# tomneda/DABstar

Hardware: AMD Instinct MI355X
Metric: DAB Mode-I ensembles/s (2.048 MS/s IQ->MSC bytes) per GPU; FIB CRC match % (higher is better)
Workload: dtype f32+i32

## Files before the change

dabstar_amd/csrc/vit_t.hip:

```cpp
#include "pipeline.h"
#include "vit_t_gen.h"
#include <vector>

namespace dabx {

__device__ __forceinline__ int bitrev4(int v) { return ((v & 1) << 3) | ((v & 2) << 1) | ((v & 4) >> 1) | ((v & 8) >> 3); }

constexpr int PJB = 32;
constexpr int PCH = 64;
constexpr int PJS = 16 * PCH + 4;
__device__ __forceinline__ int msc_class_of_group(const MscLaunch &L, int g)
{
  int c = 0;
  while (c + 1 < L.n && g >= L.c[c + 1].g0) c++;
  return c;
}

__device__ __forceinline__ uint32_t prep_ld(const uint32_t *p)
{
#if DABX_PREP_NT & 1
  return __builtin_nontemporal_load(p);
#else
  return *p;
#endif
}
__device__ __forceinline__ void prep_st(uint32_t *p, uint32_t v)
{
#if DABX_PREP_NT & 2
  __builtin_nontemporal_store(v, p);
#else
  *p = v;
#endif
}
constexpr int PREP_STG = PJB * 16 * (PCH / 4) / 256;
__device__ __forceinline__ void prep_item(int it, int cw, bool full, int &d, int &pl, int &job)
{
  int jp;
  if (full) { d = it & (PCH / 4 - 1); jp = it / (PCH / 4); }
  else { d = it % cw; jp = it / cw; }
  pl = jp & 15; job = jp >> 4;
}
__device__ __forceinline__ void prep_request(uint32_t (&stage)[PREP_STG], int tid, int p0, int cw, const uint8_t *const *s_base, const long long *s_r,
                                             const int2 *s_mv )
{
  const bool full = cw == PCH / 4;
  if (full) {
    const int pl = (tid >> 4) & 15, d = tid & 15;
    const int brev = bitrev4(pl);
    const unsigned in_plane = (unsigned)pl * (CIF_BITS / 16) + (unsigned)p0 + 4u * (unsigned)d;
#pragma unroll
    for (int r = 0; r < PREP_STG; r++) {
      const uint8_t *base = s_base[r];
      uint32_t v = 0x7F7F7F7Fu;
      if (base) {
        const unsigned slot = (unsigned)(s_r[r] - 16 + brev) & (TDI_SLOTS - 1);
        const int2 mv = s_mv[r];
        v = prep_ld(reinterpret_cast<const uint32_t *>(base + (brev < mv.x ? mv.y : 0) + (size_t)slot * CIF_BITS + in_plane));
      }
      stage[r] = v;
    }
    return;
  }
#pragma unroll
  for (int r = 0; r < PREP_STG; r++) {
    const int it = tid + 256 * r;
    uint32_t v = 0x7F7F7F7Fu;
    if (it < PJB * 16 * cw) {
      int d, pl, job;
      prep_item(it, cw, full, d, pl, job);
      const uint8_t *base = s_base[job];
      if (base) {
        const long long cif = s_r[job] - 16 + bitrev4(pl);
        const int2 mv = s_mv[job];
        v = prep_ld(reinterpret_cast<const uint32_t *>(base + (bitrev4(pl) < mv.x ? mv.y : 0) + (size_t)(cif & (TDI_SLOTS - 1)) * CIF_BITS + (size_t)pl * (CIF_BITS / 16) + p0 + 4 * d));
      }
    }
    stage[r] = v;
  }
}

__global__ __launch_bounds__(256) void k_msc_prep(EngineDev e, int cifs, MscLaunch L)
{
  __builtin_amdgcn_s_setprio(3);
  __shared__ __attribute__((aligned(16))) uint8_t tile[PJB * PJS];
  __shared__ const uint8_t *s_base[PJB];
  __shared__ long long s_r[PJB];
  __shared__ int2 s_mv[PJB];
  const int ci = msc_class_of_group(L, blockIdx.x / (64 / PJB));
  const MscLaunchCls &cl = L.c[ci];
  const int n_in = cl.n_in;
  uint32_t *inT = cl.inT;
  const int tid = threadIdx.x, job0 = (blockIdx.x - cl.g0 * (64 / PJB)) * PJB;
  if (tid < PJB) {
    const MscJob q = msc_class_job(e, cl, job0 + tid, cifs);
    const SubchDev &sc = e.subch[(size_t)q.s * e.max_subch + q.j];
    s_base[tid] = q.valid ? e.tdi + (size_t)q.s * TDI_SLOTS * CIF_BITS + sc.cu_start * 4 : nullptr;
    s_r[tid] = q.r;
    s_mv[tid] = make_int2(q.valid ? msc_move_thr(sc, q.r) : 0, (sc.prev_cu_start - sc.cu_start) * 4);
  }
  const int rows = n_in / 4 + 1;
  const int jl = tid & (PJB - 1), pg = (tid >> 5) & 3, qd = tid >> 7;
  uint32_t *dst = inT + (size_t)(job0 >> 6) * rows * 64 + (job0 & 63) + jl;
  if (pg == 0 && qd == 0) dst[(size_t)(rows - 1) * 64] = 0x7F7F7F7Fu;
  __syncthreads();
  const int npos = n_in / 16;
  uint32_t stage[PREP_STG];
  auto chunk_dwords = [&](int p0) { return (npos - p0 < PCH ? npos - p0 : PCH) / 4; };
  if (npos > 0) prep_request(stage, tid, 0, chunk_dwords(0), s_base, s_r, s_mv);
  for (int p0 = 0; p0 < npos; p0 += PCH) {
    const int cw = chunk_dwords(p0);
    const bool full = cw == PCH / 4;
    if (full) {
      uint8_t *mine_w = tile + ((tid >> 4) & 15) * PCH + 4 * (tid & 15);
#pragma unroll
      for (int r = 0; r < PREP_STG; r++) *reinterpret_cast<uint32_t *>(mine_w + r * PJS) = stage[r];
    } else {
#pragma unroll
      for (int r = 0; r < PREP_STG; r++) {
        const int it = tid + 256 * r;
        if (it < PJB * 16 * cw) {
          int d, pl, job;
          prep_item(it, cw, full, d, pl, job);
          *reinterpret_cast<uint32_t *>(tile + job * PJS + pl * PCH + 4 * d) = stage[r];
        }
      }
    }
    __syncthreads();
    if (p0 + PCH < npos) prep_request(stage, tid, p0 + PCH, chunk_dwords(p0 + PCH), s_base, s_r, s_mv);
    const uint8_t *mine = tile + jl * PJS + (4 * pg) * PCH;
    for (int d = qd; d < cw; d += 2) {
      const uint32_t m0 = *reinterpret_cast<const uint32_t *>(mine + 0 * PCH + 4 * d), m1 = *reinterpret_cast<const uint32_t *>(mine + 1 * PCH + 4 * d);
      const uint32_t m2 = *reinterpret_cast<const uint32_t *>(mine + 2 * PCH + 4 * d), m3 = *reinterpret_cast<const uint32_t *>(mine + 3 * PCH + 4 * d);
      const uint32_t a = __builtin_amdgcn_perm(m1, m0, 0x05010400u), b = __builtin_amdgcn_perm(m1, m0, 0x07030602u);
      const uint32_t c = __builtin_amdgcn_perm(m3, m2, 0x05010400u), f = __builtin_amdgcn_perm(m3, m2, 0x07030602u);
      const int P = p0 + 4 * d;
      prep_st(&dst[(size_t)(4 * (P + 0) + pg) * 64], __builtin_amdgcn_perm(c, a, 0x05040100u));
      prep_st(&dst[(size_t)(4 * (P + 1) + pg) * 64], __builtin_amdgcn_perm(c, a, 0x07060302u));
      prep_st(&dst[(size_t)(4 * (P + 2) + pg) * 64], __builtin_amdgcn_perm(f, b, 0x05040100u));
      prep_st(&dst[(size_t)(4 * (P + 3) + pg) * 64], __builtin_amdgcn_perm(f, b, 0x07060302u));
    }
    __syncthreads();
  }
}

struct VtCycle { uint32_t w[24]; unsigned long long sh; };

typedef unsigned vt_u2 __attribute__((ext_vector_type(2)));
typedef const __attribute__((address_space(4))) vt_u2 *vt_cmap;

typedef __amdgpu_buffer_rsrc_t vt_rsrc;
__device__ __forceinline__ vt_rsrc vt_make_rsrc(const uint32_t *base, unsigned bytes)
{
  return __builtin_amdgcn_make_buffer_rsrc(const_cast<uint32_t *>(base), 0, (int)bytes, 0x00020000);
}
struct VtDec {
  uint2 *p;
#if DABX_VIT_BUF
  vt_rsrc rs;
  int voff;
#endif
};
__device__ __forceinline__ VtDec vt_make_dec(uint2 *group_base, int nsteps, int lane)
{
  VtDec d;
  d.p = group_base + lane;
#if DABX_VIT_BUF
  d.rs = vt_make_rsrc(reinterpret_cast<const uint32_t *>(group_base), (unsigned)nsteps * 512u);
  d.voff = lane * 8;
#else
  (void)nsteps;
#endif
  return d;
}
#ifndef DABX_VIT_ST_AUX
#define DABX_VIT_ST_AUX 2
#define DABX_VIT_LD_AUX 2
#endif
typedef unsigned vt_u2v __attribute__((ext_vector_type(2)));
__device__ __forceinline__ void vt_dec_store(const VtDec &d, int t, unsigned acc0, unsigned acc1)
{
#if DABX_VIT_BUF
  vt_u2v v; v.x = acc0; v.y = acc1;
  __builtin_amdgcn_raw_buffer_store_b64(v, d.rs, d.voff, t * 512, DABX_VIT_ST_AUX);
#elif DABX_VIT_NT & 1
  vt_u2v v; v.x = acc0; v.y = acc1;
  __builtin_nontemporal_store(v, reinterpret_cast<vt_u2v *>(&d.p[(size_t)t * 64]));
#else
  d.p[(size_t)t * 64] = make_uint2(acc0, acc1);
#endif
}
__device__ __forceinline__ uint2 vt_dec_load(const VtDec &d, int t)
{
#if DABX_VIT_BUF
  const vt_u2v v = __builtin_amdgcn_raw_buffer_load_b64(d.rs, d.voff, t * 512, DABX_VIT_LD_AUX);
  return make_uint2(v.x, v.y);
#elif DABX_VIT_NT & 2
  const vt_u2v v = __builtin_nontemporal_load(reinterpret_cast<const vt_u2v *>(&d.p[(size_t)t * 64]));
  return make_uint2(v.x, v.y);
#else
  return d.p[(size_t)t * 64];
#endif
}
#if DABX_VIT_NT & 4
constexpr int VT_IN_AUX = 2;
#else
constexpr int VT_IN_AUX = 0;
#endif
__device__ __forceinline__ void vt_fetch(VtCycle &c, vt_rsrc in_grp, int lane, vt_cmap map, int t0)
{
  c.sh = 0;
#pragma unroll
  for (int s6 = 0; s6 < 6; s6++) {
    const vt_u2 m = map[t0 + s6];
    const unsigned idx[4] = {m.x & 0xFFFFu, m.x >> 16, m.y & 0xFFFFu, m.y >> 16};
#pragma unroll
    for (int p = 0; p < 4; p++) {
      c.w[4 * s6 + p] = (uint32_t)__builtin_amdgcn_raw_buffer_load_b32(in_grp, lane * 4, (int)((idx[p] >> 2) * 256u), VT_IN_AUX);
      c.sh |= (unsigned long long)(idx[p] & 3) << (2 * (4 * s6 + p));
    }
  }
}

template <int TIE> struct VtTie { static constexpr int LIMTOP = 0, REN2 = 0; };
template <> struct VtTie<1> { static constexpr int LIMTOP = 2 * 65535, REN2 = 2 * 60000; };
template <> struct VtTie<2> { static constexpr int LIMTOP = 2 * 32767, REN2 = 2 * 30000; };

template <int C, int TIE = 0, bool CLAMP = false>
__device__ __forceinline__ void vt_one(vt::s2 (&R)[32], const VtCycle &cy, int t, const VtDec &dec_lane, vt::s2 v2n, int &Coff)
{
  unsigned w[4], b[4];
#pragma unroll
  for (int p = 0; p < 4; p++) {
    w[p] = cy.w[4 * C + p];
    b[p] = (unsigned)((cy.sh >> (2 * (4 * C + p))) & 3);
  }
  vt::s2 M[4];
  unsigned acc0, acc1;
  bool pre = false;
  vt::s2 lim = vt::pk(0, 0);
  if constexpr (TIE != 0) {
    if constexpr ((C & 1) != 0) pre = (int)R[0].x + Coff + 1020 * C > VtTie<TIE>::REN2;
    if constexpr (CLAMP) {
      int l = VtTie<TIE>::LIMTOP - Coff - 1020 * (C + 1);
      l = l < 32767 ? l : 32767;
      lim = vt::pk(l, l);
    }
  }
  if constexpr (C == 0) { vt::bm0(w, b, v2n, M); vt::step0<TIE, CLAMP>(R, M, acc0, acc1, lim); }
  else if constexpr (C == 1) { vt::bm1(w, b, v2n, M); vt::step1<TIE, CLAMP>(R, M, acc0, acc1, lim); }
  else if constexpr (C == 2) { vt::bm2(w, b, v2n, M); vt::step2<TIE, CLAMP>(R, M, acc0, acc1, lim); }
  else if constexpr (C == 3) { vt::bm3(w, b, v2n, M); vt::step3<TIE, CLAMP>(R, M, acc0, acc1, lim); }
  else if constexpr (C == 4) { vt::bm4(w, b, v2n, M); vt::step4<TIE, CLAMP>(R, M, acc0, acc1, lim); }
  else { vt::bm5(w, b, v2n, M); vt::step5<TIE, CLAMP>(R, M, acc0, acc1, lim); }
  vt_dec_store(dec_lane, t, acc0, acc1);
  if constexpr (TIE != 0 && (C & 1) != 0) {
    if (__builtin_amdgcn_ballot_w64(pre)) {
      const int mnv = vt::min64(R);
      if (pre) Coff = -mnv - 1020 * (C + 1);
    }
  }
}

template <int TIE, bool CLAMP>
__device__ __forceinline__ void vt_cycle6(vt::s2 (&R)[32], const VtCycle &cy, int t0, const VtDec &dec_lane, vt::s2 v2n, int &Coff)
{
  vt_one<0, TIE, CLAMP>(R, cy, t0 + 0, dec_lane, v2n, Coff);
  vt_one<1, TIE, CLAMP>(R, cy, t0 + 1, dec_lane, v2n, Coff);
  vt_one<2, TIE, CLAMP>(R, cy, t0 + 2, dec_lane, v2n, Coff);
  vt_one<3, TIE, CLAMP>(R, cy, t0 + 3, dec_lane, v2n, Coff);
  vt_one<4, TIE, CLAMP>(R, cy, t0 + 4, dec_lane, v2n, Coff);
  vt_one<5, TIE, CLAMP>(R, cy, t0 + 5, dec_lane, v2n, Coff);
}
template <int TIE, bool ALWAYS_CLAMP>
__device__ __forceinline__ void vt_cycle(vt::s2 (&R)[32], const VtCycle &cy, int t0, const VtDec &dec_lane, vt::s2 v2n, int &Coff)
{
  if constexpr (TIE == 0) vt_cycle6<0, false>(R, cy, t0, dec_lane, v2n, Coff);
  else {
    bool clamp = ALWAYS_CLAMP;
    if constexpr (!ALWAYS_CLAMP) {
      const int room = VtTie<TIE>::LIMTOP - Coff;
      if (__builtin_amdgcn_ballot_w64((int)R[0].x + 14280 + 12240 > room)) {
        const int mxv = vt::max64(R);
        clamp = __builtin_amdgcn_ballot_w64(mxv + 12240 > room) != 0;
      }
    }
    if (clamp) vt_cycle6<TIE, true>(R, cy, t0, dec_lane, v2n, Coff);
    else vt_cycle6<TIE, false>(R, cy, t0, dec_lane, v2n, Coff);
    Coff += 6 * 1020;
  }
}

struct VtDec6 { uint2 w0, w1, w2, w3, w4, w5; };
__device__ __forceinline__ VtDec6 vt_load_dec(const VtDec &dec_lane, int t0)
{
  VtDec6 d;
  d.w0 = vt_dec_load(dec_lane, t0); d.w1 = vt_dec_load(dec_lane, t0 + 1); d.w2 = vt_dec_load(dec_lane, t0 + 2);
  d.w3 = vt_dec_load(dec_lane, t0 + 3); d.w4 = vt_dec_load(dec_lane, t0 + 4); d.w5 = vt_dec_load(dec_lane, t0 + 5);
  return d;
}
template <int C>
__device__ __forceinline__ void vt_back_one(const uint2 w, int t, unsigned &L, unsigned &outw, uint32_t *out, const uint32_t *prbs,
                                            const unsigned char *pos_c)
{
  constexpr unsigned p = 5 - C;
  const unsigned pos = pos_c[L];
  const unsigned long long ww = ((unsigned long long)w.y << 32) | w.x;
  const unsigned bit = (unsigned)(ww >> pos) & 1u;
  const int qb = t - 6;
  outw |= bit << (((qb >> 3) & 3) * 8 + 7 - (qb & 7));
  L = (L & ~(1u << p)) | (bit << p);
  if ((qb & 31) == 0) {
    const unsigned pw = ((const __attribute__((address_space(4))) uint32_t *)(const void *)prbs)[qb >> 5];
    if (out) out[qb >> 5] = outw ^ pw;
    outw = 0;
  }
}

__device__ unsigned long long *g_vt_timeline = nullptr;
__device__ unsigned g_vt_timeline_cap = 0;
__device__ unsigned g_vt_timeline_n = 0;

template <int TIE, bool ALWAYS_CLAMP>
__device__ __forceinline__ void vt_decode(vt_rsrc in_grp, vt_cmap cmap, int nsteps, const VtDec &dec_lane, uint32_t *out, const uint32_t *prbs,
                                          const unsigned char (*pos_tab)[64], int lane, unsigned long long &t_forward_end, bool want_time)
{
  vt::s2 R[32];
#pragma unroll
  for (int r = 0; r < 32; r++) R[r] = vt::pk(2000, 2000);
  R[0] = vt::pk(0, 2000);
  int Coff = 0;
  const int last = nsteps - 6;
  VtCycle ca, cb;
  vt_fetch(ca, in_grp, lane, cmap, 0);
  vt_fetch(cb, in_grp, lane, cmap, 6);
  auto recentre = [&]() {
    const vt::s2 ref = vt::pk(R[0].x, R[0].x);
    if constexpr (TIE != 0) Coff += (int)R[0].x;
#pragma unroll
    for (int r = 0; r < 32; r++) R[r] = R[r] - ref;
  };
  vt::s2 v2n;
  asm volatile("v_mov_b32 %0, %1" : "=v"(v2n) : "s"(0xFFFE0002u));
  int t = 0;
  for (; t + 12 <= nsteps; t += 12) {
    recentre();
    vt_cycle<TIE, ALWAYS_CLAMP>(R, ca, t, dec_lane, v2n, Coff);
    vt_fetch(ca, in_grp, lane, cmap, t + 12 < last ? t + 12 : last);
    vt_cycle<TIE, ALWAYS_CLAMP>(R, cb, t + 6, dec_lane, v2n, Coff);
    vt_fetch(cb, in_grp, lane, cmap, t + 18 < last ? t + 18 : last);
  }
  if (t < nsteps) {
    recentre();
    vt_cycle<TIE, ALWAYS_CLAMP>(R, ca, t, dec_lane, v2n, Coff);
  }
  __builtin_amdgcn_fence(__ATOMIC_RELEASE, "workgroup");
  __builtin_amdgcn_s_waitcnt(0);
  __syncthreads();
  if (want_time) t_forward_end = __builtin_amdgcn_s_memrealtime();

  unsigned L = 0, outw = 0;
  VtDec6 cur = vt_load_dec(dec_lane, nsteps - 6);
  VtDec6 nx1 = vt_load_dec(dec_lane, nsteps - 12);
  for (int tc = nsteps - 6; tc >= 6; tc -= 6) {
    const int tf = tc - 12 > 6 ? tc - 12 : 6;
    const VtDec6 nx2 = vt_load_dec(dec_lane, tf);
    vt_back_one<5>(cur.w5, tc + 5, L, outw, out, prbs, pos_tab[5]);
    vt_back_one<4>(cur.w4, tc + 4, L, outw, out, prbs, pos_tab[4]);
    vt_back_one<3>(cur.w3, tc + 3, L, outw, out, prbs, pos_tab[3]);
    vt_back_one<2>(cur.w2, tc + 2, L, outw, out, prbs, pos_tab[2]);
    vt_back_one<1>(cur.w1, tc + 1, L, outw, out, prbs, pos_tab[1]);
    vt_back_one<0>(cur.w0, tc + 0, L, outw, out, prbs, pos_tab[0]);
    cur = nx1; nx1 = nx2;
  }
}

template <int TIE>
__device__ __forceinline__ void msc_vitT_body(const EngineDev &e, int cifs, const MscLaunch &ML, const uint32_t *prbs)
{
  __shared__ unsigned char pos_tab[6][64];
  const int lane = threadIdx.x;
  unsigned long long *const tl = g_vt_timeline;
  unsigned long long tl0 = 0, tl1 = 0;
  if (tl) tl0 = __builtin_amdgcn_s_memrealtime();
  for (int i = lane; i < 6 * 64; i += 64) pos_tab[i / 64][i % 64] = vt::VT_POS[i / 64][i % 64];
  int gg = blockIdx.x;
  {
    constexpr int ROUND = 1024;
    const int r = gg / ROUND, base = r * ROUND;
    const int len = ML.groups - base < ROUND ? ML.groups - base : ROUND;
    if (r & 1) gg = base + (len - 1 - (gg - base));
  }
  const MscLaunchCls &cl = ML.c[msc_class_of_group(ML, gg)];
  const int g = gg - cl.g0;
  const MscJob q = msc_class_job(e, cl, g * 64 + lane, cifs);
  const int nsteps = cl.nbits + 6, rows = cl.n_in / 4 + 1;
  const vt_rsrc in_grp = vt_make_rsrc(cl.inT + (size_t)g * rows * 64, (unsigned)rows * 256u);
  const VtDec dec_lane = vt_make_dec(cl.decT + (size_t)g * nsteps * 64, nsteps, lane);
  const vt_cmap cmap = (vt_cmap)(const void *)cl.map2;
  uint32_t *out = nullptr;
  if (q.valid)
    out = reinterpret_cast<uint32_t *>(e.msc_out + (((size_t)q.s * e.max_subch + q.j) * MSC_SLOTS + (size_t)(q.out_idx % MSC_SLOTS)) * e.msc_stride);
  vt_decode<TIE, false>(in_grp, cmap, nsteps, dec_lane, out, prbs, pos_tab, lane, tl1, tl != nullptr);
  if (tl && lane == 0) {
    const unsigned slot = atomicAdd(&g_vt_timeline_n, 1u);
    if (slot < g_vt_timeline_cap) {
      unsigned hw, xcc;
      asm volatile("s_getreg_b32 %0, hwreg(HW_REG_HW_ID)" : "=s"(hw));
      asm volatile("s_getreg_b32 %0, hwreg(HW_REG_XCC_ID)" : "=s"(xcc));
      unsigned long long *o = tl + (size_t)slot * 4;
      o[0] = ((unsigned long long)xcc << 32) | hw; o[1] = tl0; o[2] = tl1; o[3] = __builtin_amdgcn_s_memrealtime();
    }
  }
}
#ifdef DABX_VIT_WAVES
#define DABX_VIT_OCC __attribute__((amdgpu_waves_per_eu(DABX_VIT_WAVES, DABX_VIT_WAVES)))
#else
#define DABX_VIT_OCC
#endif
__global__ __launch_bounds__(64) DABX_VIT_OCC void k_msc_vitT(EngineDev e, int cifs, MscLaunch ML, const uint32_t *prbs) { msc_vitT_body<0>(e, cifs, ML, prbs); }
__global__ __launch_bounds__(64) void k_msc_vitT_avx2(EngineDev e, int cifs, MscLaunch ML, const uint32_t *prbs) { msc_vitT_body<1>(e, cifs, ML, prbs); }
__global__ __launch_bounds__(64) void k_msc_vitT_sse2(EngineDev e, int cifs, MscLaunch ML, const uint32_t *prbs) { msc_vitT_body<2>(e, cifs, ML, prbs); }

template <int TIE, bool ALWAYS_CLAMP>
__global__ __launch_bounds__(64) void k_vitT_stage(const uint32_t *symT, const uint16_t *map, int nbits, uint2 *decT, uint32_t *outw, const uint32_t *zeros)
{
  __shared__ unsigned char pos_tab[6][64];
  const int lane = threadIdx.x, g = blockIdx.x;
  for (int i = lane; i < 6 * 64; i += 64) pos_tab[i / 64][i % 64] = vt::VT_POS[i / 64][i % 64];
  const int nsteps = nbits + 6, rows = nsteps + 1;
  const vt_rsrc in_grp = vt_make_rsrc(symT + (size_t)g * rows * 64, (unsigned)rows * 256u);
  unsigned long long unused = 0;
  vt_decode<TIE, ALWAYS_CLAMP>(in_grp, (vt_cmap)(const void *)map, nsteps, vt_make_dec(decT + (size_t)g * nsteps * 64, nsteps, lane),
                               outw + ((size_t)g * 64 + lane) * (nbits / 32), zeros, pos_tab, lane, unused, false);
}

extern "C" int dabx_internal_vitT(const int16_t *soft, int nbits, int batch, int tie_mode, int always_clamp, uint8_t *bits)
{
  if (!soft || !bits || batch <= 0 || nbits < 96 || nbits % 96 != 0 || 4 * (nbits + 6) > 65532 || tie_mode < 0 || tie_mode > 2) {
    set_error("dabx_internal_vitT: bad argument");
    return DABX_E_ARG;
  }
  const int nsteps = nbits + 6, rows = nsteps + 1, groups = (batch + 63) / 64, nw = nbits / 32;
  std::vector<uint32_t> symT((size_t)groups * rows * 64, 0x7F7F7F7Fu);
  for (int b = 0; b < batch; b++)
    for (int r = 0; r < nsteps; r++) {
      uint32_t v = 0;
      for (int k = 0; k < 4; k++) {
        const int16_t sft = soft[(size_t)b * 4 * nsteps + 4 * r + k];
        int sy = tie_mode ? (int)sft + 127 : (int)(int16_t)(sft + 127);
        sy = sy < 0 ? 0 : (sy > 255 ? 255 : sy);
        v |= (uint32_t)sy << (8 * k);
      }
      symT[((size_t)(b / 64) * rows + r) * 64 + (b % 64)] = v;
    }
  std::vector<uint16_t> map((size_t)4 * nsteps + 64);
  for (size_t i = 0; i < map.size(); i++) map[i] = (uint16_t)(i < (size_t)4 * nsteps ? i : 4 * nsteps);
  uint32_t *d_sym = nullptr, *d_out = nullptr, *d_zero = nullptr;
  uint16_t *d_map = nullptr;
  uint2 *d_dec = nullptr;
  int rc = DABX_E_HIP;
  std::vector<uint32_t> outw((size_t)groups * 64 * nw);
  do {
    if (hipMalloc(&d_sym, symT.size() * 4) != hipSuccess || hipMalloc(&d_map, map.size() * 2) != hipSuccess ||
        hipMalloc(&d_dec, (size_t)groups * nsteps * 64 * sizeof(uint2)) != hipSuccess || hipMalloc(&d_out, outw.size() * 4) != hipSuccess ||
        hipMalloc(&d_zero, (size_t)(nw + 1) * 4) != hipSuccess) break;
    if (hipMemcpy(d_sym, symT.data(), symT.size() * 4, hipMemcpyHostToDevice) != hipSuccess) break;
    if (hipMemcpy(d_map, map.data(), map.size() * 2, hipMemcpyHostToDevice) != hipSuccess) break;
    if (hipMemset(d_zero, 0, (size_t)(nw + 1) * 4) != hipSuccess || hipMemset(d_out, 0, outw.size() * 4) != hipSuccess) break;
#define VT_STAGE(T, A) hipLaunchKernelGGL((k_vitT_stage<T, A>), dim3(groups), dim3(64), 0, 0, d_sym, d_map, nbits, d_dec, d_out, d_zero)
    if (tie_mode == 0) VT_STAGE(0, false);
    else if (tie_mode == 1) { if (always_clamp) VT_STAGE(1, true); else VT_STAGE(1, false); }
    else { if (always_clamp) VT_STAGE(2, true); else VT_STAGE(2, false); }
#undef VT_STAGE
    if (hipGetLastError() != hipSuccess || hipDeviceSynchronize() != hipSuccess) break;
    if (hipMemcpy(outw.data(), d_out, outw.size() * 4, hipMemcpyDeviceToHost) != hipSuccess) break;
    rc = 0;
  } while (false);
  (void)hipFree(d_sym); (void)hipFree(d_map); (void)hipFree(d_dec); (void)hipFree(d_out); (void)hipFree(d_zero);
  if (rc) { set_error("dabx_internal_vitT: HIP error"); return rc; }
  for (int b = 0; b < batch; b++) {
    const uint8_t *pb = reinterpret_cast<const uint8_t *>(outw.data() + (size_t)b * nw);
    for (int i = 0; i < nbits; i++) bits[(size_t)b * nbits + i] = (uint8_t)((pb[i >> 3] >> (7 - (i & 7))) & 1);
  }
  return 0;
}

extern "C" int dabx_internal_set_vt_timeline(void *buf, unsigned capacity_records)
{
  unsigned long long *p = reinterpret_cast<unsigned long long *>(buf);
  unsigned zero = 0;
  DABX_HIP(hipMemcpyToSymbol(HIP_SYMBOL(g_vt_timeline_cap), &capacity_records, sizeof(unsigned)));
  DABX_HIP(hipMemcpyToSymbol(HIP_SYMBOL(g_vt_timeline_n), &zero, sizeof(unsigned)));
  DABX_HIP(hipMemcpyToSymbol(HIP_SYMBOL(g_vt_timeline), &p, sizeof(p)));
  return 0;
}

int launch_msc_prep(const EngineDev &e, int cifs, const MscLaunch &L, hipStream_t st, Marker &mk)
{
  mk.begin(6, st);
  hipLaunchKernelGGL(k_msc_prep, dim3(L.groups * (64 / PJB)), dim3(256), 0, st, e, cifs, L);
  mk.end(6, st);
  DABX_HIP(hipGetLastError());
  return 0;
}
int launch_msc_vitT(const EngineDev &e, int cifs, const MscLaunch &L, hipStream_t st, Marker &mk)
{
  const DevTables *t;
  int rc = get_tables(&t);
  if (rc) return rc;
  mk.begin(7, st);
  const int grid = L.groups;
  if (e.tie_mode == 1) hipLaunchKernelGGL(k_msc_vitT_avx2, dim3(grid), dim3(64), 0, st, e, cifs, L, t->prbs_words);
  else if (e.tie_mode == 2) hipLaunchKernelGGL(k_msc_vitT_sse2, dim3(grid), dim3(64), 0, st, e, cifs, L, t->prbs_words);
  else hipLaunchKernelGGL(k_msc_vitT, dim3(grid), dim3(64), 0, st, e, cifs, L, t->prbs_words);
  mk.end(7, st);
  DABX_HIP(hipGetLastError());
  return 0;
}

}
```

dabstar_amd/csrc/vit_t_gen.h:

```cpp
#pragma once
#include <hip/hip_runtime.h>
namespace dabx { namespace vt {
typedef short s2 __attribute__((ext_vector_type(2)));
__device__ __forceinline__ unsigned u(s2 v) { return __builtin_bit_cast(unsigned, v); }
__device__ __forceinline__ s2 s(unsigned v) { return __builtin_bit_cast(s2, v); }
__device__ __forceinline__ s2 pk(int lo, int hi) { return s(__builtin_amdgcn_perm((unsigned)hi, (unsigned)lo, 0x05040100u)); }
__device__ __forceinline__ s2 mn(s2 a, s2 b) { return __builtin_elementwise_min(a, b); }
__device__ __forceinline__ s2 mx(s2 a, s2 b) { return __builtin_elementwise_max(a, b); }
__device__ __forceinline__ int min64(const s2 (&R)[32])
{ s2 a[16];
  for (int i = 0; i < 16; i++) a[i] = mn(R[i], R[i + 16]);
  for (int w = 8; w > 0; w >>= 1) for (int i = 0; i < w; i++) a[i] = mn(a[i], a[i + w]);
  return a[0].x < a[0].y ? (int)a[0].x : (int)a[0].y; }
__device__ __forceinline__ int max64(const s2 (&R)[32])
{ s2 a[16];
  for (int i = 0; i < 16; i++) a[i] = mx(R[i], R[i + 16]);
  for (int w = 8; w > 0; w >>= 1) for (int i = 0; i < w; i++) a[i] = mx(a[i], a[i + w]);
  return a[0].x > a[0].y ? (int)a[0].x : (int)a[0].y; }
__device__ __forceinline__ s2 mn_x(s2 a, s2 b)
{ s2 r; asm("v_pk_min_i16 %0, %1, %2 op_sel:[0,1] op_sel_hi:[1,0]" : "=v"(r) : "v"(a), "v"(b)); return r; }
__device__ __forceinline__ s2 sub_hl(s2 a, s2 b)
{ s2 r; asm("v_pk_sub_i16 %0, %1, %2 op_sel:[1,0] op_sel_hi:[0,1]" : "=v"(r) : "v"(a), "v"(b)); return r; }
__device__ __forceinline__ s2 sub_lh(s2 a, s2 b)
{ s2 r; asm("v_pk_sub_i16 %0, %1, %2 op_sel:[0,1] op_sel_hi:[1,0]" : "=v"(r) : "v"(a), "v"(b)); return r; }
__device__ __forceinline__ unsigned sg(s2 s0, s2 s1) { return __builtin_amdgcn_perm(u(s0), u(s1), 0x0B0A0908u); }
__device__ __forceinline__ unsigned sg_even(s2 dd, s2 ee) { return __builtin_amdgcn_perm(u(dd), u(ee), 0x0C0C090Au); }
__device__ __forceinline__ unsigned sg_odd(s2 dd, s2 ee) { return __builtin_amdgcn_perm(u(dd), u(ee), 0x090A0C0Cu); }
template <int K> __device__ __forceinline__ void fold(unsigned &acc, unsigned p)
{ constexpr unsigned M = 0x01010101u << K;
  if (K == 0) acc = p & M;
  else asm("v_and_or_b32 %0, %1, %2, %0" : "+v"(acc) : "v"(p), "s"(M)); }
__device__ __forceinline__ s2 swap_add(s2 a)
{ s2 r; asm("v_pk_add_u16 %0, %1, %1 op_sel:[0,1] op_sel_hi:[1,0]" : "=v"(r) : "v"(a)); return r; }
__device__ __forceinline__ s2 swap_sub(s2 a) { return sub_lh(a, a); }
__device__ __forceinline__ s2 add_lolo(s2 a, s2 b)
{ s2 r; asm("v_pk_add_u16 %0, %1, %2 op_sel:[0,0] op_sel_hi:[1,0]" : "=v"(r) : "v"(a), "v"(b)); return r; }
__device__ __forceinline__ s2 add_hihi(s2 a, s2 b)
{ s2 r; asm("v_pk_add_u16 %0, %1, %2 op_sel:[0,1] op_sel_hi:[1,1]" : "=v"(r) : "v"(a), "v"(b)); return r; }
__device__ __forceinline__ s2 mad2(s2 a, unsigned k)
{ s2 r; asm("v_pk_mad_i16 %0, %1, 2, %2 op_sel_hi:[1,0,1]" : "=v"(r) : "v"(a), "s"(k)); return r; }
__device__ __forceinline__ s2 madv(s2 a, s2 m, unsigned k)
{ s2 r; asm("v_pk_mad_i16 %0, %1, %2, %3" : "=v"(r) : "v"(a), "v"(m), "s"(k)); return r; }
__device__ __forceinline__ s2 pick(unsigned w_lo, unsigned b_lo, unsigned w_hi, unsigned b_hi)
{ return s(__builtin_amdgcn_perm(w_hi, w_lo, 0x0C000C00u | b_lo | ((4u + b_hi) << 16))); }
constexpr unsigned K_M255 = 0xFF01FF01u, K_M255_P255 = 0x00FFFF01u, K_M510 = 0xFE02FE02u, K_M510_P510 = 0x01FEFE02u;

__device__ constexpr unsigned char VT_P[6] = {5, 4, 3, 2, 1, 0};
__device__ constexpr unsigned char VT_POS[6][64] = {
  {0, 16, 1, 17, 2, 18, 3, 19, 4, 20, 5, 21, 6, 22, 7, 23, 32, 48, 33, 49, 34, 50, 35, 51, 36, 52, 37, 53, 38, 54, 39, 55, 8, 24, 9, 25, 10, 26, 11, 27, 12, 28, 13, 29, 14, 30, 15, 31, 40, 56, 41, 57, 42, 58, 43, 59, 44, 60, 45, 61, 46, 62, 47, 63},
  {16, 17, 18, 19, 20, 21, 22, 23, 48, 49, 50, 51, 52, 53, 54, 55, 0, 1, 2, 3, 4, 5, 6, 7, 32, 33, 34, 35, 36, 37, 38, 39, 24, 25, 26, 27, 28, 29, 30, 31, 56, 57, 58, 59, 60, 61, 62, 63, 8, 9, 10, 11, 12, 13, 14, 15, 40, 41, 42, 43, 44, 45, 46, 47},
  {16, 17, 18, 19, 20, 21, 22, 23, 0, 1, 2, 3, 4, 5, 6, 7, 48, 49, 50, 51, 52, 53, 54, 55, 32, 33, 34, 35, 36, 37, 38, 39, 24, 25, 26, 27, 28, 29, 30, 31, 8, 9, 10, 11, 12, 13, 14, 15, 56, 57, 58, 59, 60, 61, 62, 63, 40, 41, 42, 43, 44, 45, 46, 47},
  {16, 17, 18, 19, 0, 1, 2, 3, 20, 21, 22, 23, 4, 5, 6, 7, 48, 49, 50, 51, 32, 33, 34, 35, 52, 53, 54, 55, 36, 37, 38, 39, 24, 25, 26, 27, 8, 9, 10, 11, 28, 29, 30, 31, 12, 13, 14, 15, 56, 57, 58, 59, 40, 41, 42, 43, 60, 61, 62, 63, 44, 45, 46, 47},
  {16, 17, 0, 1, 18, 19, 2, 3, 20, 21, 4, 5, 22, 23, 6, 7, 48, 49, 32, 33, 50, 51, 34, 35, 52, 53, 36, 37, 54, 55, 38, 39, 24, 25, 8, 9, 26, 27, 10, 11, 28, 29, 12, 13, 30, 31, 14, 15, 56, 57, 40, 41, 58, 59, 42, 43, 60, 61, 44, 45, 62, 63, 46, 47},
  {16, 0, 17, 1, 18, 2, 19, 3, 20, 4, 21, 5, 22, 6, 23, 7, 48, 32, 49, 33, 50, 34, 51, 35, 52, 36, 53, 37, 54, 38, 55, 39, 24, 8, 25, 9, 26, 10, 27, 11, 28, 12, 29, 13, 30, 14, 31, 15, 56, 40, 57, 41, 58, 42, 59, 43, 60, 44, 61, 45, 62, 46, 63, 47},
};

__device__ __forceinline__ void bm0(const unsigned (&w)[4], const unsigned (&b)[4], s2 v2n, s2 (&M)[4])
{
  const s2 A = pick(w[0], b[0], w[3], b[3]);
  const s2 B = pick(w[1], b[1], w[2], b[2]);
  const s2 TS = swap_add(A);
  const s2 Y2 = mad2(TS, K_M510);
  const s2 XB = mad2(B, K_M255);
  const s2 S = swap_add(XB);
  const s2 D = swap_sub(XB);
  M[0] = Y2 + S;
  M[1] = add_lolo(Y2, D);
  M[2] = add_hihi(Y2, D);
  M[3] = Y2 - S;
}
template <int TIE = 0, bool CLAMP = false>
__device__ __forceinline__ void step0(s2 (&R)[32], const s2 (&M)[4], unsigned &acc0, unsigned &acc1, s2 lim = s2{0, 0})
{
  const s2 M0 = M[0];
  const s2 M1 = M[1];
  const s2 M2 = M[2];
  const s2 M3 = M[3];
  s2 t1_0 = R[0] + M0, t2_0 = R[0] - M0;
  if constexpr (CLAMP) { t1_0 = mn(t1_0, lim); t2_0 = mn(t2_0, lim); }
  R[0] = mn_x(t1_0, t2_0);
  s2 t1_1 = R[1] + M3, t2_1 = R[1] - M3;
  if constexpr (CLAMP) { t1_1 = mn(t1_1, lim); t2_1 = mn(t2_1, lim); }
  R[1] = mn_x(t1_1, t2_1);
  if constexpr (TIE == 1) fold<0>(acc0, sg_even(sub_lh(t1_0, t2_0), sub_hl(t2_0, t1_0)) | sg_odd(sub_lh(t1_1, t2_1), sub_hl(t2_1, t1_1)));
  else fold<0>(acc0, sg_even(sub_hl(t2_0, t1_0), sub_lh(t1_0, t2_0)) | sg_odd(sub_hl(t2_1, t1_1), sub_lh(t1_1, t2_1)));
  s2 t1_2 = R[2] - M1, t2_2 = R[2] + M1;
  if constexpr (CLAMP) { t1_2 = mn(t1_2, lim); t2_2 = mn(t2_2, lim); }
  R[2] = mn_x(t1_2, t2_2);
  s2 t1_3 = R[3] - M2, t2_3 = R[3] + M2;
  if constexpr (CLAMP) { t1_3 = mn(t1_3, lim); t2_3 = mn(t2_3, lim); }
  R[3] = mn_x(t1_3, t2_3);
  if constexpr (TIE == 1) fold<1>(acc0, sg_even(sub_lh(t1_2, t2_2), sub_hl(t2_2, t1_2)) | sg_odd(sub_lh(t1_3, t2_3), sub_hl(t2_3, t1_3)));
  else fold<1>(acc0, sg_even(sub_hl(t2_2, t1_2), sub_lh(t1_2, t2_2)) | sg_odd(sub_hl(t2_3, t1_3), sub_lh(t1_3, t2_3)));
  s2 t1_4 = R[4] - M1, t2_4 = R[4] + M1;
  if constexpr (CLAMP) { t1_4 = mn(t1_4, lim); t2_4 = mn(t2_4, lim); }
  R[4] = mn_x(t1_4, t2_4);
  s2 t1_5 = R[5] - M2, t2_5 = R[5] + M2;
  if constexpr (CLAMP) { t1_5 = mn(t1_5, lim); t2_5 = mn(t2_5, lim); }
  R[5] = mn_x(t1_5, t2_5);
  if constexpr (TIE == 1) fold<2>(acc0, sg_even(sub_lh(t1_4, t2_4), sub_hl(t2_4, t1_4)) | sg_odd(sub_lh(t1_5, t2_5), sub_hl(t2_5, t1_5)));
  else fold<2>(acc0, sg_even(sub_hl(t2_4, t1_4), sub_lh(t1_4, t2_4)) | sg_odd(sub_hl(t2_5, t1_5), sub_lh(t1_5, t2_5)));
  s2 t1_6 = R[6] + M0, t2_6 = R[6] - M0;
  if constexpr (CLAMP) { t1_6 = mn(t1_6, lim); t2_6 = mn(t2_6, lim); }
  R[6] = mn_x(t1_6, t2_6);
  s2 t1_7 = R[7] + M3, t2_7 = R[7] - M3;
  if constexpr (CLAMP) { t1_7 = mn(t1_7, lim); t2_7 = mn(t2_7, lim); }
  R[7] = mn_x(t1_7, t2_7);
  if constexpr (TIE == 1) fold<3>(acc0, sg_even(sub_lh(t1_6, t2_6), sub_hl(t2_6, t1_6)) | sg_odd(sub_lh(t1_7, t2_7), sub_hl(t2_7, t1_7)));
  else fold<3>(acc0, sg_even(sub_hl(t2_6, t1_6), sub_lh(t1_6, t2_6)) | sg_odd(sub_hl(t2_7, t1_7), sub_lh(t1_7, t2_7)));
  s2 t1_8 = R[8] + M1, t2_8 = R[8] - M1;
  if constexpr (CLAMP) { t1_8 = mn(t1_8, lim); t2_8 = mn(t2_8, lim); }
  R[8] = mn_x(t1_8, t2_8);
  s2 t1_9 = R[9] + M2, t2_9 = R[9] - M2;
  if constexpr (CLAMP) { t1_9 = mn(t1_9, lim); t2_9 = mn(t2_9, lim); }
  R[9] = mn_x(t1_9, t2_9);
  if constexpr (TIE == 1) fold<4>(acc0, sg_even(sub_lh(t1_8, t2_8), sub_hl(t2_8, t1_8)) | sg_odd(sub_lh(t1_9, t2_9), sub_hl(t2_9, t1_9)));
  else fold<4>(acc0, sg_even(sub_hl(t2_8, t1_8), sub_lh(t1_8, t2_8)) | sg_odd(sub_hl(t2_9, t1_9), sub_lh(t1_9, t2_9)));
  s2 t1_10 = R[10] - M0, t2_10 = R[10] + M0;
  if constexpr (CLAMP) { t1_10 = mn(t1_10, lim); t2_10 = mn(t2_10, lim); }
  R[10] = mn_x(t1_10, t2_10);
  s2 t1_11 = R[11] - M3, t2_11 = R[11] + M3;
  if constexpr (CLAMP) { t1_11 = mn(t1_11, lim); t2_11 = mn(t2_11, lim); }
  R[11] = mn_x(t1_11, t2_11);
  if constexpr (TIE == 1) fold<5>(acc0, sg_even(sub_lh(t1_10, t2_10), sub_hl(t2_10, t1_10)) | sg_odd(sub_lh(t1_11, t2_11), sub_hl(t2_11, t1_11)));
  else fold<5>(acc0, sg_even(sub_hl(t2_10, t1_10), sub_lh(t1_10, t2_10)) | sg_odd(sub_hl(t2_11, t1_11), sub_lh(t1_11, t2_11)));
  s2 t1_12 = R[12] - M0, t2_12 = R[12] + M0;
  if constexpr (CLAMP) { t1_12 = mn(t1_12, lim); t2_12 = mn(t2_12, lim); }
  R[12] = mn_x(t1_12, t2_12);
  s2 t1_13 = R[13] - M3, t2_13 = R[13] + M3;
  if constexpr (CLAMP) { t1_13 = mn(t1_13, lim); t2_13 = mn(t2_13, lim); }
  R[13] = mn_x(t1_13, t2_13);
  if constexpr (TIE == 1) fold<6>(acc0, sg_even(sub_lh(t1_12, t2_12), sub_hl(t2_12, t1_12)) | sg_odd(sub_lh(t1_13, t2_13), sub_hl(t2_13, t1_13)));
  else fold<6>(acc0, sg_even(sub_hl(t2_12, t1_12), sub_lh(t1_12, t2_12)) | sg_odd(sub_hl(t2_13, t1_13), sub_lh(t1_13, t2_13)));
  s2 t1_14 = R[14] + M1, t2_14 = R[14] - M1;
  if constexpr (CLAMP) { t1_14 = mn(t1_14, lim); t2_14 = mn(t2_14, lim); }
  R[14] = mn_x(t1_14, t2_14);
  s2 t1_15 = R[15] + M2, t2_15 = R[15] - M2;
  if constexpr (CLAMP) { t1_15 = mn(t1_15, lim); t2_15 = mn(t2_15, lim); }
  R[15] = mn_x(t1_15, t2_15);
  if constexpr (TIE == 1) fold<7>(acc0, sg_even(sub_lh(t1_14, t2_14), sub_hl(t2_14, t1_14)) | sg_odd(sub_lh(t1_15, t2_15), sub_hl(t2_15, t1_15)));
  else fold<7>(acc0, sg_even(sub_hl(t2_14, t1_14), sub_lh(t1_14, t2_14)) | sg_odd(sub_hl(t2_15, t1_15), sub_lh(t1_15, t2_15)));
  s2 t1_16 = R[16] - M3, t2_16 = R[16] + M3;
  if constexpr (CLAMP) { t1_16 = mn(t1_16, lim); t2_16 = mn(t2_16, lim); }
  R[16] = mn_x(t1_16, t2_16);
  s2 t1_17 = R[17] - M0, t2_17 = R[17] + M0;
  if constexpr (CLAMP) { t1_17 = mn(t1_17, lim); t2_17 = mn(t2_17, lim); }
  R[17] = mn_x(t1_17, t2_17);
  if constexpr (TIE == 1) fold<0>(acc1, sg_even(sub_lh(t1_16, t2_16), sub_hl(t2_16, t1_16)) | sg_odd(sub_lh(t1_17, t2_17), sub_hl(t2_17, t1_17)));
  else fold<0>(acc1, sg_even(sub_hl(t2_16, t1_16), sub_lh(t1_16, t2_16)) | sg_odd(sub_hl(t2_17, t1_17), sub_lh(t1_17, t2_17)));
  s2 t1_18 = R[18] + M2, t2_18 = R[18] - M2;
  if constexpr (CLAMP) { t1_18 = mn(t1_18, lim); t2_18 = mn(t2_18, lim); }
  R[18] = mn_x(t1_18, t2_18);
  s2 t1_19 = R[19] + M1, t2_19 = R[19] - M1;
  if constexpr (CLAMP) { t1_19 = mn(t1_19, lim); t2_19 = mn(t2_19, lim); }
  R[19] = mn_x(t1_19, t2_19);
  if constexpr (TIE == 1) fold<1>(acc1, sg_even(sub_lh(t1_18, t2_18), sub_hl(t2_18, t1_18)) | sg_odd(sub_lh(t1_19, t2_19), sub_hl(t2_19, t1_19)));
  else fold<1>(acc1, sg_even(sub_hl(t2_18, t1_18), sub_lh(t1_18, t2_18)) | sg_odd(sub_hl(t2_19, t1_19), sub_lh(t1_19, t2_19)));
  s2 t1_20 = R[20] + M2, t2_20 = R[20] - M2;
  if constexpr (CLAMP) { t1_20 = mn(t1_20, lim); t2_20 = mn(t2_20, lim); }
  R[20] = mn_x(t1_20, t2_20);
  s2 t1_21 = R[21] + M1, t2_21 = R[21] - M1;
  if constexpr (CLAMP) { t1_21 = mn(t1_21, lim); t2_21 = mn(t2_21, lim); }
  R[21] = mn_x(t1_21, t2_21);
  if constexpr (TIE == 1) fold<2>(acc1, sg_even(sub_lh(t1_20, t2_20), sub_hl(t2_20, t1_20)) | sg_odd(sub_lh(t1_21, t2_21), sub_hl(t2_21, t1_21)));
  else fold<2>(acc1, sg_even(sub_hl(t2_20, t1_20), sub_lh(t1_20, t2_20)) | sg_odd(sub_hl(t2_21, t1_21), sub_lh(t1_21, t2_21)));
  s2 t1_22 = R[22] - M3, t2_22 = R[22] + M3;
  if constexpr (CLAMP) { t1_22 = mn(t1_22, lim); t2_22 = mn(t2_22, lim); }
  R[22] = mn_x(t1_22, t2_22);
  s2 t1_23 = R[23] - M0, t2_23 = R[23] + M0;
  if constexpr (CLAMP) { t1_23 = mn(t1_23, lim); t2_23 = mn(t2_23, lim); }
  R[23] = mn_x(t1_23, t2_23);
  if constexpr (TIE == 1) fold<3>(acc1, sg_even(sub_lh(t1_22, t2_22), sub_hl(t2_22, t1_22)) | sg_odd(sub_lh(t1_23, t2_23), sub_hl(t2_23, t1_23)));
  else fold<3>(acc1, sg_even(sub_hl(t2_22, t1_22), sub_lh(t1_22, t2_22)) | sg_odd(sub_hl(t2_23, t1_23), sub_lh(t1_23, t2_23)));
  s2 t1_24 = R[24] - M2, t2_24 = R[24] + M2;
  if constexpr (CLAMP) { t1_24 = mn(t1_24, lim); t2_24 = mn(t2_24, lim); }
  R[24] = mn_x(t1_24, t2_24);
  s2 t1_25 = R[25] - M1, t2_25 = R[25] + M1;
  if constexpr (CLAMP) { t1_25 = mn(t1_25, lim); t2_25 = mn(t2_25, lim); }
  R[25] = mn_x(t1_25, t2_25);
  if constexpr (TIE == 1) fold<4>(acc1, sg_even(sub_lh(t1_24, t2_24), sub_hl(t2_24, t1_24)) | sg_odd(sub_lh(t1_25, t2_25), sub_hl(t2_25, t1_25)));
  else fold<4>(acc1, sg_even(sub_hl(t2_24, t1_24), sub_lh(t1_24, t2_24)) | sg_odd(sub_hl(t2_25, t1_25), sub_lh(t1_25, t2_25)));
  s2 t1_26 = R[26] + M3, t2_26 = R[26] - M3;
  if constexpr (CLAMP) { t1_26 = mn(t1_26, lim); t2_26 = mn(t2_26, lim); }
  R[26] = mn_x(t1_26, t2_26);
  s2 t1_27 = R[27] + M0, t2_27 = R[27] - M0;
  if constexpr (CLAMP) { t1_27 = mn(t1_27, lim); t2_27 = mn(t2_27, lim); }
  R[27] = mn_x(t1_27, t2_27);
  if constexpr (TIE == 1) fold<5>(acc1, sg_even(sub_lh(t1_26, t2_26), sub_hl(t2_26, t1_26)) | sg_odd(sub_lh(t1_27, t2_27), sub_hl(t2_27, t1_27)));
  else fold<5>(acc1, sg_even(sub_hl(t2_26, t1_26), sub_lh(t1_26, t2_26)) | sg_odd(sub_hl(t2_27, t1_27), sub_lh(t1_27, t2_27)));
  s2 t1_28 = R[28] + M3, t2_28 = R[28] - M3;
  if constexpr (CLAMP) { t1_28 = mn(t1_28, lim); t2_28 = mn(t2_28, lim); }
  R[28] = mn_x(t1_28, t2_28);
  s2 t1_29 = R[29] + M0, t2_29 = R[29] - M0;
  if constexpr (CLAMP) { t1_29 = mn(t1_29, lim); t2_29 = mn(t2_29, lim); }
  R[29] = mn_x(t1_29, t2_29);
  if constexpr (TIE == 1) fold<6>(acc1, sg_even(sub_lh(t1_28, t2_28), sub_hl(t2_28, t1_28)) | sg_odd(sub_lh(t1_29, t2_29), sub_hl(t2_29, t1_29)));
  else fold<6>(acc1, sg_even(sub_hl(t2_28, t1_28), sub_lh(t1_28, t2_28)) | sg_odd(sub_hl(t2_29, t1_29), sub_lh(t1_29, t2_29)));
  s2 t1_30 = R[30] - M2, t2_30 = R[30] + M2;
  if constexpr (CLAMP) { t1_30 = mn(t1_30, lim); t2_30 = mn(t2_30, lim); }
  R[30] = mn_x(t1_30, t2_30);
  s2 t1_31 = R[31] - M1, t2_31 = R[31] + M1;
  if constexpr (CLAMP) { t1_31 = mn(t1_31, lim); t2_31 = mn(t2_31, lim); }
  R[31] = mn_x(t1_31, t2_31);
  if constexpr (TIE == 1) fold<7>(acc1, sg_even(sub_lh(t1_30, t2_30), sub_hl(t2_30, t1_30)) | sg_odd(sub_lh(t1_31, t2_31), sub_hl(t2_31, t1_31)));
  else fold<7>(acc1, sg_even(sub_hl(t2_30, t1_30), sub_lh(t1_30, t2_30)) | sg_odd(sub_hl(t2_31, t1_31), sub_lh(t1_31, t2_31)));
  if constexpr (TIE == 1) { acc0 = ~acc0; acc1 = ~acc1; }
}

__device__ __forceinline__ void bm1(const unsigned (&w)[4], const unsigned (&b)[4], s2 v2n, s2 (&M)[4])
{
  const s2 A = pick(w[0], b[0], w[3], b[3]);
  const s2 U1 = pick(w[1], b[1], w[1], b[1]);
  const s2 U2 = pick(w[2], b[2], w[2], b[2]);
  const s2 TS = swap_add(A);
  const s2 Y2 = mad2(TS, K_M510);
  const s2 X1N = madv(U1, v2n, K_M255_P255);
  const s2 X2N = madv(U2, v2n, K_M255_P255);
  const s2 SN = X1N + X2N;
  const s2 DN = X1N - X2N;
  M[0] = Y2 + SN;
  M[1] = Y2 + DN;
  M[2] = Y2 - SN;
  M[3] = Y2 - DN;
}
template <int TIE = 0, bool CLAMP = false>
__device__ __forceinline__ void step1(s2 (&R)[32], const s2 (&M)[4], unsigned &acc0, unsigned &acc1, s2 lim = s2{0, 0})
{
  const s2 M0 = M[0];
  const s2 M1 = M[1];
  const s2 M2 = M[2];
  const s2 M3 = M[3];
  { s2 a0 = R[0] + M0, b0 = R[16] - M0, a1 = R[0] - M0, b1 = R[16] + M0;
    if constexpr (CLAMP) { a0 = mn(a0, lim); b0 = mn(b0, lim); a1 = mn(a1, lim); b1 = mn(b1, lim); }
    R[0] = mn(a0, b0); R[16] = mn(a1, b1);
    if constexpr (TIE == 1) fold<0>(acc0, sg(a0 - b0, a1 - b1)); else fold<0>(acc0, sg(b0 - a0, b1 - a1)); }
  { s2 a0 = R[1] - M1, b0 = R[17] + M1, a1 = R[1] + M1, b1 = R[17] - M1;
    if constexpr (CLAMP) { a0 = mn(a0, lim); b0 = mn(b0, lim); a1 = mn(a1, lim); b1 = mn(b1, lim); }
    R[1] = mn(a0, b0); R[17] = mn(a1, b1);
    if constexpr (TIE == 1) fold<1>(acc0, sg(a0 - b0, a1 - b1)); else fold<1>(acc0, sg(b0 - a0, b1 - a1)); }
  { s2 a0 = R[2] - M1, b0 = R[18] + M1, a1 = R[2] + M1, b1 = R[18] - M1;
    if constexpr (CLAMP) { a0 = mn(a0, lim); b0 = mn(b0, lim); a1 = mn(a1, lim); b1 = mn(b1, lim); }
    R[2] = mn(a0, b0); R[18] = mn(a1, b1);
    if constexpr (TIE == 1) fold<2>(acc0, sg(a0 - b0, a1 - b1)); else fold<2>(acc0, sg(b0 - a0, b1 - a1)); }
  { s2 a0 = R[3] + M0, b0 = R[19] - M0, a1 = R[3] - M0, b1 = R[19] + M0;
    if constexpr (CLAMP) { a0 = mn(a0, lim); b0 = mn(b0, lim); a1 = mn(a1, lim); b1 = mn(b1, lim); }
    R[3] = mn(a0, b0); R[19] = mn(a1, b1);
    if constexpr (TIE == 1) fold<3>(acc0, sg(a0 - b0, a1 - b1)); else fold<3>(acc0, sg(b0 - a0, b1 - a1)); }
  { s2 a0 = R[4] + M1, b0 = R[20] - M1, a1 = R[4] - M1, b1 = R[20] + M1;
    if constexpr (CLAMP) { a0 = mn(a0, lim); b0 = mn(b0, lim); a1 = mn(a1, lim); b1 = mn(b1, lim); }
    R[4] = mn(a0, b0); R[20] = mn(a1, b1);
    if constexpr (TIE == 1) fold<4>(acc0, sg(a0 - b0, a1 - b1)); else fold<4>(acc0, sg(b0 - a0, b1 - a1)); }
  { s2 a0 = R[5] - M0, b0 = R[21] + M0, a1 = R[5] + M0, b1 = R[21] - M0;
    if constexpr (CLAMP) { a0 = mn(a0, lim); b0 = mn(b0, lim); a1 = mn(a1, lim); b1 = mn(b1, lim); }
    R[5] = mn(a0, b0); R[21] = mn(a1, b1);
    if constexpr (TIE == 1) fold<5>(acc0, sg(a0 - b0, a1 - b1)); else fold<5>(acc0, sg(b0 - a0, b1 - a1)); }
  { s2 a0 = R[6] - M0, b0 = R[22] + M0, a1 = R[6] + M0, b1 = R[22] - M0;
    if constexpr (CLAMP) { a0 = mn(a0, lim); b0 = mn(b0, lim); a1 = mn(a1, lim); b1 = mn(b1, lim); }
    R[6] = mn(a0, b0); R[22] = mn(a1, b1);
    if constexpr (TIE == 1) fold<6>(acc0, sg(a0 - b0, a1 - b1)); else fold<6>(acc0, sg(b0 - a0, b1 - a1)); }
  { s2 a0 = R[7] + M1, b0 = R[23] - M1, a1 = R[7] - M1, b1 = R[23] + M1;
    if constexpr (CLAMP) { a0 = mn(a0, lim); b0 = mn(b0, lim); a1 = mn(a1, lim); b1 = mn(b1, lim); }
    R[7] = mn(a0, b0); R[23] = mn(a1, b1);
    if constexpr (TIE == 1) fold<7>(acc0, sg(a0 - b0, a1 - b1)); else fold<7>(acc0, sg(b0 - a0, b1 - a1)); }
  { s2 a0 = R[8] - M2, b0 = R[24] + M2, a1 = R[8] + M2, b1 = R[24] - M2;
    if constexpr (CLAMP) { a0 = mn(a0, lim); b0 = mn(b0, lim); a1 = mn(a1, lim); b1 = mn(b1, lim); }
    R[8] = mn(a0, b0); R[24] = mn(a1, b1);
    if constexpr (TIE == 1) fold<0>(acc1, sg(a0 - b0, a1 - b1)); else fold<0>(acc1, sg(b0 - a0, b1 - a1)); }
  { s2 a0 = R[9] + M3, b0 = R[25] - M3, a1 = R[9] - M3, b1 = R[25] + M3;
    if constexpr (CLAMP) { a0 = mn(a0, lim); b0 = mn(b0, lim); a1 = mn(a1, lim); b1 = mn(b1, lim); }
    R[9] = mn(a0, b0); R[25] = mn(a1, b1);
    if constexpr (TIE == 1) fold<1>(acc1, sg(a0 - b0, a1 - b1)); else fold<1>(acc1, sg(b0 - a0, b1 - a1)); }
  { s2 a0 = R[10] + M3, b0 = R[26] - M3, a1 = R[10] - M3, b1 = R[26] + M3;
    if constexpr (CLAMP) { a0 = mn(a0, lim); b0 = mn(b0, lim); a1 = mn(a1, lim); b1 = mn(b1, lim); }
    R[10] = mn(a0, b0); R[26] = mn(a1, b1);
    if constexpr (TIE == 1) fold<2>(acc1, sg(a0 - b0, a1 - b1)); else fold<2>(acc1, sg(b0 - a0, b1 - a1)); }
  { s2 a0 = R[11] - M2, b0 = R[27] + M2, a1 = R[11] + M2, b1 = R[27] - M2;
    if constexpr (CLAMP) { a0 = mn(a0, lim); b0 = mn(b0, lim); a1 = mn(a1, lim); b1 = mn(b1, lim); }
    R[11] = mn(a0, b0); R[27] = mn(a1, b1);
    if constexpr (TIE == 1) fold<3>(acc1, sg(a0 - b0, a1 - b1)); else fold<3>(acc1, sg(b0 - a0, b1 - a1)); }
  { s2 a0 = R[12] - M3, b0 = R[28] + M3, a1 = R[12] + M3, b1 = R[28] - M3;
    if constexpr (CLAMP) { a0 = mn(a0, lim); b0 = mn(b0, lim); a1 = mn(a1, lim); b1 = mn(b1, lim); }
    R[12] = mn(a0, b0); R[28] = mn(a1, b1);
    if constexpr (TIE == 1) fold<4>(acc1, sg(a0 - b0, a1 - b1)); else fold<4>(acc1, sg(b0 - a0, b1 - a1)); }
  { s2 a0 = R[13] + M2, b0 = R[29] - M2, a1 = R[13] - M2, b1 = R[29] + M2;
    if constexpr (CLAMP) { a0 = mn(a0, lim); b0 = mn(b0, lim); a1 = mn(a1, lim); b1 = mn(b1, lim); }
    R[13] = mn(a0, b0); R[29] = mn(a1, b1);
    if constexpr (TIE == 1) fold<5>(acc1, sg(a0 - b0, a1 - b1)); else fold<5>(acc1, sg(b0 - a0, b1 - a1)); }
  { s2 a0 = R[14] + M2, b0 = R[30] - M2, a1 = R[14] - M2, b1 = R[30] + M2;
    if constexpr (CLAMP) { a0 = mn(a0, lim); b0 = mn(b0, lim); a1 = mn(a1, lim); b1 = mn(b1, lim); }
    R[14] = mn(a0, b0); R[30] = mn(a1, b1);
    if constexpr (TIE == 1) fold<6>(acc1, sg(a0 - b0, a1 - b1)); else fold<6>(acc1, sg(b0 - a0, b1 - a1)); }
  { s2 a0 = R[15] - M3, b0 = R[31] + M3, a1 = R[15] + M3, b1 = R[31] - M3;
    if constexpr (CLAMP) { a0 = mn(a0, lim); b0 = mn(b0, lim); a1 = mn(a1, lim); b1 = mn(b1, lim); }
    R[15] = mn(a0, b0); R[31] = mn(a1, b1);
    if constexpr (TIE == 1) fold<7>(acc1, sg(a0 - b0, a1 - b1)); else fold<7>(acc1, sg(b0 - a0, b1 - a1)); }
  if constexpr (TIE == 1) { acc0 = ~acc0; acc1 = ~acc1; }
}

__device__ __forceinline__ void bm2(const unsigned (&w)[4], const unsigned (&b)[4], s2 v2n, s2 (&M)[4])
{
  const s2 A = pick(w[0], b[0], w[3], b[3]);
  const s2 U1 = pick(w[1], b[1], w[1], b[1]);
  const s2 U2 = pick(w[2], b[2], w[2], b[2]);
  const s2 TS = swap_add(A);
  const s2 YN = madv(TS, v2n, K_M510_P510);
  const s2 X1N = madv(U1, v2n, K_M255_P255);
  const s2 X2 = mad2(U2, K_M255);
  const s2 PN = YN + X1N;
  const s2 QN = YN - X1N;
  M[0] = PN + X2;
  M[1] = PN - X2;
  M[2] = QN - X2;
  M[3] = QN + X2;
}
template <int TIE = 0, bool CLAMP = false>
__device__ __forceinline__ void step2(s2 (&R)[32], const s2 (&M)[4], unsigned &acc0, unsigned &acc1, s2 lim = s2{0, 0})
{
  const s2 M0 = M[0];
  const s2 M1 = M[1];
  const s2 M2 = M[2];
  const s2 M3 = M[3];
  { s2 a0 = R[0] + M0, b0 = R[8] - M0, a1 = R[0] - M0, b1 = R[8] + M0;
    if constexpr (CLAMP) { a0 = mn(a0, lim); b0 = mn(b0, lim); a1 = mn(a1, lim); b1 = mn(b1, lim); }
    R[0] = mn(a0, b0); R[8] = mn(a1, b1);
    if constexpr (TIE == 1) fold<0>(acc0, sg(a0 - b0, a1 - b1)); else fold<0>(acc0, sg(b0 - a0, b1 - a1)); }
  { s2 a0 = R[1] - M1, b0 = R[9] + M1, a1 = R[1] + M1, b1 = R[9] - M1;
    if constexpr (CLAMP) { a0 = mn(a0, lim); b0 = mn(b0, lim); a1 = mn(a1, lim); b1 = mn(b1, lim); }
    R[1] = mn(a0, b0); R[9] = mn(a1, b1);
    if constexpr (TIE == 1) fold<1>(acc0, sg(a0 - b0, a1 - b1)); else fold<1>(acc0, sg(b0 - a0, b1 - a1)); }
  { s2 a0 = R[2] + M1, b0 = R[10] - M1, a1 = R[2] - M1, b1 = R[10] + M1;
    if constexpr (CLAMP) { a0 = mn(a0, lim); b0 = mn(b0, lim); a1 = mn(a1, lim); b1 = mn(b1, lim); }
    R[2] = mn(a0, b0); R[10] = mn(a1, b1);
    if constexpr (TIE == 1) fold<2>(acc0, sg(a0 - b0, a1 - b1)); else fold<2>(acc0, sg(b0 - a0, b1 - a1)); }
  { s2 a0 = R[3] - M0, b0 = R[11] + M0, a1 = R[3] + M0, b1 = R[11] - M0;
    if constexpr (CLAMP) { a0 = mn(a0, lim); b0 = mn(b0, lim); a1 = mn(a1, lim); b1 = mn(b1, lim); }
    R[3] = mn(a0, b0); R[11] = mn(a1, b1);
    if constexpr (TIE == 1) fold<3>(acc0, sg(a0 - b0, a1 - b1)); else fold<3>(acc0, sg(b0 - a0, b1 - a1)); }
  { s2 a0 = R[4] - M2, b0 = R[12] + M2, a1 = R[4] + M2, b1 = R[12] - M2;
    if constexpr (CLAMP) { a0 = mn(a0, lim); b0 = mn(b0, lim); a1 = mn(a1, lim); b1 = mn(b1, lim); }
    R[4] = mn(a0, b0); R[12] = mn(a1, b1);
    if constexpr (TIE == 1) fold<4>(acc0, sg(a0 - b0, a1 - b1)); else fold<4>(acc0, sg(b0 - a0, b1 - a1)); }
  { s2 a0 = R[5] + M3, b0 = R[13] - M3, a1 = R[5] - M3, b1 = R[13] + M3;
    if constexpr (CLAMP) { a0 = mn(a0, lim); b0 = mn(b0, lim); a1 = mn(a1, lim); b1 = mn(b1, lim); }
    R[5] = mn(a0, b0); R[13] = mn(a1, b1);
    if constexpr (TIE == 1) fold<5>(acc0, sg(a0 - b0, a1 - b1)); else fold<5>(acc0, sg(b0 - a0, b1 - a1)); }
  { s2 a0 = R[6] - M3, b0 = R[14] + M3, a1 = R[6] + M3, b1 = R[14] - M3;
    if constexpr (CLAMP) { a0 = mn(a0, lim); b0 = mn(b0, lim); a1 = mn(a1, lim); b1 = mn(b1, lim); }
    R[6] = mn(a0, b0); R[14] = mn(a1, b1);
    if constexpr (TIE == 1) fold<6>(acc0, sg(a0 - b0, a1 - b1)); else fold<6>(acc0, sg(b0 - a0, b1 - a1)); }
  { s2 a0 = R[7] + M2, b0 = R[15] - M2, a1 = R[7] - M2, b1 = R[15] + M2;
    if constexpr (CLAMP) { a0 = mn(a0, lim); b0 = mn(b0, lim); a1 = mn(a1, lim); b1 = mn(b1, lim); }
    R[7] = mn(a0, b0); R[15] = mn(a1, b1);
    if constexpr (TIE == 1) fold<7>(acc0, sg(a0 - b0, a1 - b1)); else fold<7>(acc0, sg(b0 - a0, b1 - a1)); }
  { s2 a0 = R[16] + M2, b0 = R[24] - M2, a1 = R[16] - M2, b1 = R[24] + M2;
    if constexpr (CLAMP) { a0 = mn(a0, lim); b0 = mn(b0, lim); a1 = mn(a1, lim); b1 = mn(b1, lim); }
    R[16] = mn(a0, b0); R[24] = mn(a1, b1);
    if constexpr (TIE == 1) fold<0>(acc1, sg(a0 - b0, a1 - b1)); else fold<0>(acc1, sg(b0 - a0, b1 - a1)); }
  { s2 a0 = R[17] - M3, b0 = R[25] + M3, a1 = R[17] + M3, b1 = R[25] - M3;
    if constexpr (CLAMP) { a0 = mn(a0, lim); b0 = mn(b0, lim); a1 = mn(a1, lim); b1 = mn(b1, lim); }
    R[17] = mn(a0, b0); R[25] = mn(a1, b1);
    if constexpr (TIE == 1) fold<1>(acc1, sg(a0 - b0, a1 - b1)); else fold<1>(acc1, sg(b0 - a0, b1 - a1)); }
  { s2 a0 = R[18] + M3, b0 = R[26] - M3, a1 = R[18] - M3, b1 = R[26] + M3;
    if constexpr (CLAMP) { a0 = mn(a0, lim); b0 = mn(b0, lim); a1 = mn(a1, lim); b1 = mn(b1, lim); }
    R[18] = mn(a0, b0); R[26] = mn(a1, b1);
    if constexpr (TIE == 1) fold<2>(acc1, sg(a0 - b0, a1 - b1)); else fold<2>(acc1, sg(b0 - a0, b1 - a1)); }
  { s2 a0 = R[19] - M2, b0 = R[27] + M2, a1 = R[19] + M2, b1 = R[27] - M2;
    if constexpr (CLAMP) { a0 = mn(a0, lim); b0 = mn(b0, lim); a1 = mn(a1, lim); b1 = mn(b1, lim); }
    R[19] = mn(a0, b0); R[27] = mn(a1, b1);
    if constexpr (TIE == 1) fold<3>(acc1, sg(a0 - b0, a1 - b1)); else fold<3>(acc1, sg(b0 - a0, b1 - a1)); }
  { s2 a0 = R[20] - M0, b0 = R[28] + M0, a1 = R[20] + M0, b1 = R[28] - M0;
    if constexpr (CLAMP) { a0 = mn(a0, lim); b0 = mn(b0, lim); a1 = mn(a1, lim); b1 = mn(b1, lim); }
    R[20] = mn(a0, b0); R[28] = mn(a1, b1);
    if constexpr (TIE == 1) fold<4>(acc1, sg(a0 - b0, a1 - b1)); else fold<4>(acc1, sg(b0 - a0, b1 - a1)); }
  { s2 a0 = R[21] + M1, b0 = R[29] - M1, a1 = R[21] - M1, b1 = R[29] + M1;
    if constexpr (CLAMP) { a0 = mn(a0, lim); b0 = mn(b0, lim); a1 = mn(a1, lim); b1 = mn(b1, lim); }
    R[21] = mn(a0, b0); R[29] = mn(a1, b1);
    if constexpr (TIE == 1) fold<5>(acc1, sg(a0 - b0, a1 - b1)); else fold<5>(acc1, sg(b0 - a0, b1 - a1)); }
  { s2 a0 = R[22] - M1, b0 = R[30] + M1, a1 = R[22] + M1, b1 = R[30] - M1;
    if constexpr (CLAMP) { a0 = mn(a0, lim); b0 = mn(b0, lim); a1 = mn(a1, lim); b1 = mn(b1, lim); }
    R[22] = mn(a0, b0); R[30] = mn(a1, b1);
    if constexpr (TIE == 1) fold<6>(acc1, sg(a0 - b0, a1 - b1)); else fold<6>(acc1, sg(b0 - a0, b1 - a1)); }
  { s2 a0 = R[23] + M0, b0 = R[31] - M0, a1 = R[23] - M0, b1 = R[31] + M0;
    if constexpr (CLAMP) { a0 = mn(a0, lim); b0 = mn(b0, lim); a1 = mn(a1, lim); b1 = mn(b1, lim); }
    R[23] = mn(a0, b0); R[31] = mn(a1, b1);
    if constexpr (TIE == 1) fold<7>(acc1, sg(a0 - b0, a1 - b1)); else fold<7>(acc1, sg(b0 - a0, b1 - a1)); }
  if constexpr (TIE == 1) { acc0 = ~acc0; acc1 = ~acc1; }
}

__device__ __forceinline__ void bm3(const unsigned (&w)[4], const unsigned (&b)[4], s2 v2n, s2 (&M)[4])
{
  const s2 A = pick(w[0], b[0], w[3], b[3]);
  const s2 U1 = pick(w[1], b[1], w[1], b[1]);
  const s2 U2 = pick(w[2], b[2], w[2], b[2]);
  const s2 TS = swap_add(A);
  const s2 YN = madv(TS, v2n, K_M510_P510);
  const s2 X1N = madv(U1, v2n, K_M255_P255);
  const s2 X2 = mad2(U2, K_M255);
  const s2 PN = YN + X1N;
  const s2 QN = YN - X1N;
  M[0] = PN + X2;
  M[1] = PN - X2;
  M[2] = QN - X2;
  M[3] = QN + X2;
}
template <int TIE = 0, bool CLAMP = false>
__device__ __forceinline__ void step3(s2 (&R)[32], const s2 (&M)[4], unsigned &acc0, unsigned &acc1, s2 lim = s2{0, 0})
{
  const s2 M0 = M[0];
  const s2 M1 = M[1];
  const s2 M2 = M[2];
  const s2 M3 = M[3];
  { s2 a0 = R[0] + M0, b0 = R[4] - M0, a1 = R[0] - M0, b1 = R[4] + M0;
    if constexpr (CLAMP) { a0 = mn(a0, lim); b0 = mn(b0, lim); a1 = mn(a1, lim); b1 = mn(b1, lim); }
    R[0] = mn(a0, b0); R[4] = mn(a1, b1);
    if constexpr (TIE == 1) fold<0>(acc0, sg(a0 - b0, a1 - b1)); else fold<0>(acc0, sg(b0 - a0, b1 - a1)); }
  { s2 a0 = R[1] + M1, b0 = R[5] - M1, a1 = R[1] - M1, b1 = R[5] + M1;
    if constexpr (CLAMP) { a0 = mn(a0, lim); b0 = mn(b0, lim); a1 = mn(a1, lim); b1 = mn(b1, lim); }
    R[1] = mn(a0, b0); R[5] = mn(a1, b1);
    if constexpr (TIE == 1) fold<1>(acc0, sg(a0 - b0, a1 - b1)); else fold<1>(acc0, sg(b0 - a0, b1 - a1)); }
  { s2 a0 = R[2] - M2, b0 = R[6] + M2, a1 = R[2] + M2, b1 = R[6] - M2;
    if constexpr (CLAMP) { a0 = mn(a0, lim); b0 = mn(b0, lim); a1 = mn(a1, lim); b1 = mn(b1, lim); }
    R[2] = mn(a0, b0); R[6] = mn(a1, b1);
    if constexpr (TIE == 1) fold<2>(acc0, sg(a0 - b0, a1 - b1)); else fold<2>(acc0, sg(b0 - a0, b1 - a1)); }
  { s2 a0 = R[3] - M3, b0 = R[7] + M3, a1 = R[3] + M3, b1 = R[7] - M3;
    if constexpr (CLAMP) { a0 = mn(a0, lim); b0 = mn(b0, lim); a1 = mn(a1, lim); b1 = mn(b1, lim); }
    R[3] = mn(a0, b0); R[7] = mn(a1, b1);
    if constexpr (TIE == 1) fold<3>(acc0, sg(a0 - b0, a1 - b1)); else fold<3>(acc0, sg(b0 - a0, b1 - a1)); }
  { s2 a0 = R[8] + M2, b0 = R[12] - M2, a1 = R[8] - M2, b1 = R[12] + M2;
    if constexpr (CLAMP) { a0 = mn(a0, lim); b0 = mn(b0, lim); a1 = mn(a1, lim); b1 = mn(b1, lim); }
    R[8] = mn(a0, b0); R[12] = mn(a1, b1);
    if constexpr (TIE == 1) fold<4>(acc0, sg(a0 - b0, a1 - b1)); else fold<4>(acc0, sg(b0 - a0, b1 - a1)); }
  { s2 a0 = R[9] + M3, b0 = R[13] - M3, a1 = R[9] - M3, b1 = R[13] + M3;
    if constexpr (CLAMP) { a0 = mn(a0, lim); b0 = mn(b0, lim); a1 = mn(a1, lim); b1 = mn(b1, lim); }
    R[9] = mn(a0, b0); R[13] = mn(a1, b1);
    if constexpr (TIE == 1) fold<5>(acc0, sg(a0 - b0, a1 - b1)); else fold<5>(acc0, sg(b0 - a0, b1 - a1)); }
  { s2 a0 = R[10] - M0, b0 = R[14] + M0, a1 = R[10] + M0, b1 = R[14] - M0;
    if constexpr (CLAMP) { a0 = mn(a0, lim); b0 = mn(b0, lim); a1 = mn(a1, lim); b1 = mn(b1, lim); }
    R[10] = mn(a0, b0); R[14] = mn(a1, b1);
    if constexpr (TIE == 1) fold<6>(acc0, sg(a0 - b0, a1 - b1)); else fold<6>(acc0, sg(b0 - a0, b1 - a1)); }
  { s2 a0 = R[11] - M1, b0 = R[15] + M1, a1 = R[11] + M1, b1 = R[15] - M1;
    if constexpr (CLAMP) { a0 = mn(a0, lim); b0 = mn(b0, lim); a1 = mn(a1, lim); b1 = mn(b1, lim); }
    R[11] = mn(a0, b0); R[15] = mn(a1, b1);
    if constexpr (TIE == 1) fold<7>(acc0, sg(a0 - b0, a1 - b1)); else fold<7>(acc0, sg(b0 - a0, b1 - a1)); }
  { s2 a0 = R[16] - M1, b0 = R[20] + M1, a1 = R[16] + M1, b1 = R[20] - M1;
    if constexpr (CLAMP) { a0 = mn(a0, lim); b0 = mn(b0, lim); a1 = mn(a1, lim); b1 = mn(b1, lim); }
    R[16] = mn(a0, b0); R[20] = mn(a1, b1);
    if constexpr (TIE == 1) fold<0>(acc1, sg(a0 - b0, a1 - b1)); else fold<0>(acc1, sg(b0 - a0, b1 - a1)); }
  { s2 a0 = R[17] - M0, b0 = R[21] + M0, a1 = R[17] + M0, b1 = R[21] - M0;
    if constexpr (CLAMP) { a0 = mn(a0, lim); b0 = mn(b0, lim); a1 = mn(a1, lim); b1 = mn(b1, lim); }
    R[17] = mn(a0, b0); R[21] = mn(a1, b1);
    if constexpr (TIE == 1) fold<1>(acc1, sg(a0 - b0, a1 - b1)); else fold<1>(acc1, sg(b0 - a0, b1 - a1)); }
  { s2 a0 = R[18] + M3, b0 = R[22] - M3, a1 = R[18] - M3, b1 = R[22] + M3;
    if constexpr (CLAMP) { a0 = mn(a0, lim); b0 = mn(b0, lim); a1 = mn(a1, lim); b1 = mn(b1, lim); }
    R[18] = mn(a0, b0); R[22] = mn(a1, b1);
    if constexpr (TIE == 1) fold<2>(acc1, sg(a0 - b0, a1 - b1)); else fold<2>(acc1, sg(b0 - a0, b1 - a1)); }
  { s2 a0 = R[19] + M2, b0 = R[23] - M2, a1 = R[19] - M2, b1 = R[23] + M2;
    if constexpr (CLAMP) { a0 = mn(a0, lim); b0 = mn(b0, lim); a1 = mn(a1, lim); b1 = mn(b1, lim); }
    R[19] = mn(a0, b0); R[23] = mn(a1, b1);
    if constexpr (TIE == 1) fold<3>(acc1, sg(a0 - b0, a1 - b1)); else fold<3>(acc1, sg(b0 - a0, b1 - a1)); }
  { s2 a0 = R[24] - M3, b0 = R[28] + M3, a1 = R[24] + M3, b1 = R[28] - M3;
    if constexpr (CLAMP) { a0 = mn(a0, lim); b0 = mn(b0, lim); a1 = mn(a1, lim); b1 = mn(b1, lim); }
    R[24] = mn(a0, b0); R[28] = mn(a1, b1);
    if constexpr (TIE == 1) fold<4>(acc1, sg(a0 - b0, a1 - b1)); else fold<4>(acc1, sg(b0 - a0, b1 - a1)); }
  { s2 a0 = R[25] - M2, b0 = R[29] + M2, a1 = R[25] + M2, b1 = R[29] - M2;
    if constexpr (CLAMP) { a0 = mn(a0, lim); b0 = mn(b0, lim); a1 = mn(a1, lim); b1 = mn(b1, lim); }
    R[25] = mn(a0, b0); R[29] = mn(a1, b1);
    if constexpr (TIE == 1) fold<5>(acc1, sg(a0 - b0, a1 - b1)); else fold<5>(acc1, sg(b0 - a0, b1 - a1)); }
  { s2 a0 = R[26] + M1, b0 = R[30] - M1, a1 = R[26] - M1, b1 = R[30] + M1;
    if constexpr (CLAMP) { a0 = mn(a0, lim); b0 = mn(b0, lim); a1 = mn(a1, lim); b1 = mn(b1, lim); }
    R[26] = mn(a0, b0); R[30] = mn(a1, b1);
    if constexpr (TIE == 1) fold<6>(acc1, sg(a0 - b0, a1 - b1)); else fold<6>(acc1, sg(b0 - a0, b1 - a1)); }
  { s2 a0 = R[27] + M0, b0 = R[31] - M0, a1 = R[27] - M0, b1 = R[31] + M0;
    if constexpr (CLAMP) { a0 = mn(a0, lim); b0 = mn(b0, lim); a1 = mn(a1, lim); b1 = mn(b1, lim); }
    R[27] = mn(a0, b0); R[31] = mn(a1, b1);
    if constexpr (TIE == 1) fold<7>(acc1, sg(a0 - b0, a1 - b1)); else fold<7>(acc1, sg(b0 - a0, b1 - a1)); }
  if constexpr (TIE == 1) { acc0 = ~acc0; acc1 = ~acc1; }
}

__device__ __forceinline__ void bm4(const unsigned (&w)[4], const unsigned (&b)[4], s2 v2n, s2 (&M)[4])
{
  const s2 A = pick(w[0], b[0], w[3], b[3]);
  const s2 U1 = pick(w[1], b[1], w[1], b[1]);
  const s2 U2 = pick(w[2], b[2], w[2], b[2]);
  const s2 TS = swap_add(A);
  const s2 Y2 = mad2(TS, K_M510);
  const s2 X1 = mad2(U1, K_M255);
  const s2 X2N = madv(U2, v2n, K_M255_P255);
  const s2 PP = Y2 + X1;
  const s2 QQ = Y2 - X1;
  M[0] = PP + X2N;
  M[1] = QQ - X2N;
  M[2] = PP - X2N;
  M[3] = QQ + X2N;
}
template <int TIE = 0, bool CLAMP = false>
__device__ __forceinline__ void step4(s2 (&R)[32], const s2 (&M)[4], unsigned &acc0, unsigned &acc1, s2 lim = s2{0, 0})
{
  const s2 M0 = M[0];
  const s2 M1 = M[1];
  const s2 M2 = M[2];
  const s2 M3 = M[3];
  { s2 a0 = R[0] + M0, b0 = R[2] - M0, a1 = R[0] - M0, b1 = R[2] + M0;
    if constexpr (CLAMP) { a0 = mn(a0, lim); b0 = mn(b0, lim); a1 = mn(a1, lim); b1 = mn(b1, lim); }
    R[0] = mn(a0, b0); R[2] = mn(a1, b1);
    if constexpr (TIE == 1) fold<0>(acc0, sg(a0 - b0, a1 - b1)); else fold<0>(acc0, sg(b0 - a0, b1 - a1)); }
  { s2 a0 = R[1] - M1, b0 = R[3] + M1, a1 = R[1] + M1, b1 = R[3] - M1;
    if constexpr (CLAMP) { a0 = mn(a0, lim); b0 = mn(b0, lim); a1 = mn(a1, lim); b1 = mn(b1, lim); }
    R[1] = mn(a0, b0); R[3] = mn(a1, b1);
    if constexpr (TIE == 1) fold<1>(acc0, sg(a0 - b0, a1 - b1)); else fold<1>(acc0, sg(b0 - a0, b1 - a1)); }
  { s2 a0 = R[4] + M1, b0 = R[6] - M1, a1 = R[4] - M1, b1 = R[6] + M1;
    if constexpr (CLAMP) { a0 = mn(a0, lim); b0 = mn(b0, lim); a1 = mn(a1, lim); b1 = mn(b1, lim); }
    R[4] = mn(a0, b0); R[6] = mn(a1, b1);
    if constexpr (TIE == 1) fold<2>(acc0, sg(a0 - b0, a1 - b1)); else fold<2>(acc0, sg(b0 - a0, b1 - a1)); }
  { s2 a0 = R[5] - M0, b0 = R[7] + M0, a1 = R[5] + M0, b1 = R[7] - M0;
    if constexpr (CLAMP) { a0 = mn(a0, lim); b0 = mn(b0, lim); a1 = mn(a1, lim); b1 = mn(b1, lim); }
    R[5] = mn(a0, b0); R[7] = mn(a1, b1);
    if constexpr (TIE == 1) fold<3>(acc0, sg(a0 - b0, a1 - b1)); else fold<3>(acc0, sg(b0 - a0, b1 - a1)); }
  { s2 a0 = R[8] - M2, b0 = R[10] + M2, a1 = R[8] + M2, b1 = R[10] - M2;
    if constexpr (CLAMP) { a0 = mn(a0, lim); b0 = mn(b0, lim); a1 = mn(a1, lim); b1 = mn(b1, lim); }
    R[8] = mn(a0, b0); R[10] = mn(a1, b1);
    if constexpr (TIE == 1) fold<4>(acc0, sg(a0 - b0, a1 - b1)); else fold<4>(acc0, sg(b0 - a0, b1 - a1)); }
  { s2 a0 = R[9] + M3, b0 = R[11] - M3, a1 = R[9] - M3, b1 = R[11] + M3;
    if constexpr (CLAMP) { a0 = mn(a0, lim); b0 = mn(b0, lim); a1 = mn(a1, lim); b1 = mn(b1, lim); }
    R[9] = mn(a0, b0); R[11] = mn(a1, b1);
    if constexpr (TIE == 1) fold<5>(acc0, sg(a0 - b0, a1 - b1)); else fold<5>(acc0, sg(b0 - a0, b1 - a1)); }
  { s2 a0 = R[12] - M3, b0 = R[14] + M3, a1 = R[12] + M3, b1 = R[14] - M3;
    if constexpr (CLAMP) { a0 = mn(a0, lim); b0 = mn(b0, lim); a1 = mn(a1, lim); b1 = mn(b1, lim); }
    R[12] = mn(a0, b0); R[14] = mn(a1, b1);
    if constexpr (TIE == 1) fold<6>(acc0, sg(a0 - b0, a1 - b1)); else fold<6>(acc0, sg(b0 - a0, b1 - a1)); }
  { s2 a0 = R[13] + M2, b0 = R[15] - M2, a1 = R[13] - M2, b1 = R[15] + M2;
    if constexpr (CLAMP) { a0 = mn(a0, lim); b0 = mn(b0, lim); a1 = mn(a1, lim); b1 = mn(b1, lim); }
    R[13] = mn(a0, b0); R[15] = mn(a1, b1);
    if constexpr (TIE == 1) fold<7>(acc0, sg(a0 - b0, a1 - b1)); else fold<7>(acc0, sg(b0 - a0, b1 - a1)); }
  { s2 a0 = R[16] - M2, b0 = R[18] + M2, a1 = R[16] + M2, b1 = R[18] - M2;
    if constexpr (CLAMP) { a0 = mn(a0, lim); b0 = mn(b0, lim); a1 = mn(a1, lim); b1 = mn(b1, lim); }
    R[16] = mn(a0, b0); R[18] = mn(a1, b1);
    if constexpr (TIE == 1) fold<0>(acc1, sg(a0 - b0, a1 - b1)); else fold<0>(acc1, sg(b0 - a0, b1 - a1)); }
  { s2 a0 = R[17] + M3, b0 = R[19] - M3, a1 = R[17] - M3, b1 = R[19] + M3;
    if constexpr (CLAMP) { a0 = mn(a0, lim); b0 = mn(b0, lim); a1 = mn(a1, lim); b1 = mn(b1, lim); }
    R[17] = mn(a0, b0); R[19] = mn(a1, b1);
    if constexpr (TIE == 1) fold<1>(acc1, sg(a0 - b0, a1 - b1)); else fold<1>(acc1, sg(b0 - a0, b1 - a1)); }
  { s2 a0 = R[20] - M3, b0 = R[22] + M3, a1 = R[20] + M3, b1 = R[22] - M3;
    if constexpr (CLAMP) { a0 = mn(a0, lim); b0 = mn(b0, lim); a1 = mn(a1, lim); b1 = mn(b1, lim); }
    R[20] = mn(a0, b0); R[22] = mn(a1, b1);
    if constexpr (TIE == 1) fold<2>(acc1, sg(a0 - b0, a1 - b1)); else fold<2>(acc1, sg(b0 - a0, b1 - a1)); }
  { s2 a0 = R[21] + M2, b0 = R[23] - M2, a1 = R[21] - M2, b1 = R[23] + M2;
    if constexpr (CLAMP) { a0 = mn(a0, lim); b0 = mn(b0, lim); a1 = mn(a1, lim); b1 = mn(b1, lim); }
    R[21] = mn(a0, b0); R[23] = mn(a1, b1);
    if constexpr (TIE == 1) fold<3>(acc1, sg(a0 - b0, a1 - b1)); else fold<3>(acc1, sg(b0 - a0, b1 - a1)); }
  { s2 a0 = R[24] + M0, b0 = R[26] - M0, a1 = R[24] - M0, b1 = R[26] + M0;
    if constexpr (CLAMP) { a0 = mn(a0, lim); b0 = mn(b0, lim); a1 = mn(a1, lim); b1 = mn(b1, lim); }
    R[24] = mn(a0, b0); R[26] = mn(a1, b1);
    if constexpr (TIE == 1) fold<4>(acc1, sg(a0 - b0, a1 - b1)); else fold<4>(acc1, sg(b0 - a0, b1 - a1)); }
  { s2 a0 = R[25] - M1, b0 = R[27] + M1, a1 = R[25] + M1, b1 = R[27] - M1;
    if constexpr (CLAMP) { a0 = mn(a0, lim); b0 = mn(b0, lim); a1 = mn(a1, lim); b1 = mn(b1, lim); }
    R[25] = mn(a0, b0); R[27] = mn(a1, b1);
    if constexpr (TIE == 1) fold<5>(acc1, sg(a0 - b0, a1 - b1)); else fold<5>(acc1, sg(b0 - a0, b1 - a1)); }
  { s2 a0 = R[28] + M1, b0 = R[30] - M1, a1 = R[28] - M1, b1 = R[30] + M1;
    if constexpr (CLAMP) { a0 = mn(a0, lim); b0 = mn(b0, lim); a1 = mn(a1, lim); b1 = mn(b1, lim); }
    R[28] = mn(a0, b0); R[30] = mn(a1, b1);
    if constexpr (TIE == 1) fold<6>(acc1, sg(a0 - b0, a1 - b1)); else fold<6>(acc1, sg(b0 - a0, b1 - a1)); }
  { s2 a0 = R[29] - M0, b0 = R[31] + M0, a1 = R[29] + M0, b1 = R[31] - M0;
    if constexpr (CLAMP) { a0 = mn(a0, lim); b0 = mn(b0, lim); a1 = mn(a1, lim); b1 = mn(b1, lim); }
    R[29] = mn(a0, b0); R[31] = mn(a1, b1);
    if constexpr (TIE == 1) fold<7>(acc1, sg(a0 - b0, a1 - b1)); else fold<7>(acc1, sg(b0 - a0, b1 - a1)); }
  if constexpr (TIE == 1) { acc0 = ~acc0; acc1 = ~acc1; }
}

__device__ __forceinline__ void bm5(const unsigned (&w)[4], const unsigned (&b)[4], s2 v2n, s2 (&M)[4])
{
  const s2 A = pick(w[0], b[0], w[3], b[3]);
  const s2 U1 = pick(w[1], b[1], w[1], b[1]);
  const s2 U2 = pick(w[2], b[2], w[2], b[2]);
  const s2 TS = swap_add(A);
  const s2 YN = madv(TS, v2n, K_M510_P510);
  const s2 X1 = mad2(U1, K_M255);
  const s2 X2 = mad2(U2, K_M255);
  const s2 SS = X1 + X2;
  const s2 DD = X1 - X2;
  M[0] = YN + SS;
  M[1] = YN - SS;
  M[2] = YN + DD;
  M[3] = YN - DD;
}
template <int TIE = 0, bool CLAMP = false>
__device__ __forceinline__ void step5(s2 (&R)[32], const s2 (&M)[4], unsigned &acc0, unsigned &acc1, s2 lim = s2{0, 0})
{
  const s2 M0 = M[0];
  const s2 M1 = M[1];
  const s2 M2 = M[2];
  const s2 M3 = M[3];
  { s2 a0 = R[0] + M0, b0 = R[1] - M0, a1 = R[0] - M0, b1 = R[1] + M0;
    if constexpr (CLAMP) { a0 = mn(a0, lim); b0 = mn(b0, lim); a1 = mn(a1, lim); b1 = mn(b1, lim); }
    R[0] = mn(a0, b0); R[1] = mn(a1, b1);
    if constexpr (TIE == 1) fold<0>(acc0, sg(a0 - b0, a1 - b1)); else fold<0>(acc0, sg(b0 - a0, b1 - a1)); }
  { s2 a0 = R[2] + M1, b0 = R[3] - M1, a1 = R[2] - M1, b1 = R[3] + M1;
    if constexpr (CLAMP) { a0 = mn(a0, lim); b0 = mn(b0, lim); a1 = mn(a1, lim); b1 = mn(b1, lim); }
    R[2] = mn(a0, b0); R[3] = mn(a1, b1);
    if constexpr (TIE == 1) fold<1>(acc0, sg(a0 - b0, a1 - b1)); else fold<1>(acc0, sg(b0 - a0, b1 - a1)); }
  { s2 a0 = R[4] - M2, b0 = R[5] + M2, a1 = R[4] + M2, b1 = R[5] - M2;
    if constexpr (CLAMP) { a0 = mn(a0, lim); b0 = mn(b0, lim); a1 = mn(a1, lim); b1 = mn(b1, lim); }
    R[4] = mn(a0, b0); R[5] = mn(a1, b1);
    if constexpr (TIE == 1) fold<2>(acc0, sg(a0 - b0, a1 - b1)); else fold<2>(acc0, sg(b0 - a0, b1 - a1)); }
  { s2 a0 = R[6] - M3, b0 = R[7] + M3, a1 = R[6] + M3, b1 = R[7] - M3;
    if constexpr (CLAMP) { a0 = mn(a0, lim); b0 = mn(b0, lim); a1 = mn(a1, lim); b1 = mn(b1, lim); }
    R[6] = mn(a0, b0); R[7] = mn(a1, b1);
    if constexpr (TIE == 1) fold<3>(acc0, sg(a0 - b0, a1 - b1)); else fold<3>(acc0, sg(b0 - a0, b1 - a1)); }
  { s2 a0 = R[8] - M2, b0 = R[9] + M2, a1 = R[8] + M2, b1 = R[9] - M2;
    if constexpr (CLAMP) { a0 = mn(a0, lim); b0 = mn(b0, lim); a1 = mn(a1, lim); b1 = mn(b1, lim); }
    R[8] = mn(a0, b0); R[9] = mn(a1, b1);
    if constexpr (TIE == 1) fold<4>(acc0, sg(a0 - b0, a1 - b1)); else fold<4>(acc0, sg(b0 - a0, b1 - a1)); }
  { s2 a0 = R[10] - M3, b0 = R[11] + M3, a1 = R[10] + M3, b1 = R[11] - M3;
    if constexpr (CLAMP) { a0 = mn(a0, lim); b0 = mn(b0, lim); a1 = mn(a1, lim); b1 = mn(b1, lim); }
    R[10] = mn(a0, b0); R[11] = mn(a1, b1);
    if constexpr (TIE == 1) fold<5>(acc0, sg(a0 - b0, a1 - b1)); else fold<5>(acc0, sg(b0 - a0, b1 - a1)); }
  { s2 a0 = R[12] + M0, b0 = R[13] - M0, a1 = R[12] - M0, b1 = R[13] + M0;
    if constexpr (CLAMP) { a0 = mn(a0, lim); b0 = mn(b0, lim); a1 = mn(a1, lim); b1 = mn(b1, lim); }
    R[12] = mn(a0, b0); R[13] = mn(a1, b1);
    if constexpr (TIE == 1) fold<6>(acc0, sg(a0 - b0, a1 - b1)); else fold<6>(acc0, sg(b0 - a0, b1 - a1)); }
  { s2 a0 = R[14] + M1, b0 = R[15] - M1, a1 = R[14] - M1, b1 = R[15] + M1;
    if constexpr (CLAMP) { a0 = mn(a0, lim); b0 = mn(b0, lim); a1 = mn(a1, lim); b1 = mn(b1, lim); }
    R[14] = mn(a0, b0); R[15] = mn(a1, b1);
    if constexpr (TIE == 1) fold<7>(acc0, sg(a0 - b0, a1 - b1)); else fold<7>(acc0, sg(b0 - a0, b1 - a1)); }
  { s2 a0 = R[16] + M2, b0 = R[17] - M2, a1 = R[16] - M2, b1 = R[17] + M2;
    if constexpr (CLAMP) { a0 = mn(a0, lim); b0 = mn(b0, lim); a1 = mn(a1, lim); b1 = mn(b1, lim); }
    R[16] = mn(a0, b0); R[17] = mn(a1, b1);
    if constexpr (TIE == 1) fold<0>(acc1, sg(a0 - b0, a1 - b1)); else fold<0>(acc1, sg(b0 - a0, b1 - a1)); }
  { s2 a0 = R[18] + M3, b0 = R[19] - M3, a1 = R[18] - M3, b1 = R[19] + M3;
    if constexpr (CLAMP) { a0 = mn(a0, lim); b0 = mn(b0, lim); a1 = mn(a1, lim); b1 = mn(b1, lim); }
    R[18] = mn(a0, b0); R[19] = mn(a1, b1);
    if constexpr (TIE == 1) fold<1>(acc1, sg(a0 - b0, a1 - b1)); else fold<1>(acc1, sg(b0 - a0, b1 - a1)); }
  { s2 a0 = R[20] - M0, b0 = R[21] + M0, a1 = R[20] + M0, b1 = R[21] - M0;
    if constexpr (CLAMP) { a0 = mn(a0, lim); b0 = mn(b0, lim); a1 = mn(a1, lim); b1 = mn(b1, lim); }
    R[20] = mn(a0, b0); R[21] = mn(a1, b1);
    if constexpr (TIE == 1) fold<2>(acc1, sg(a0 - b0, a1 - b1)); else fold<2>(acc1, sg(b0 - a0, b1 - a1)); }
  { s2 a0 = R[22] - M1, b0 = R[23] + M1, a1 = R[22] + M1, b1 = R[23] - M1;
    if constexpr (CLAMP) { a0 = mn(a0, lim); b0 = mn(b0, lim); a1 = mn(a1, lim); b1 = mn(b1, lim); }
    R[22] = mn(a0, b0); R[23] = mn(a1, b1);
    if constexpr (TIE == 1) fold<3>(acc1, sg(a0 - b0, a1 - b1)); else fold<3>(acc1, sg(b0 - a0, b1 - a1)); }
  { s2 a0 = R[24] - M0, b0 = R[25] + M0, a1 = R[24] + M0, b1 = R[25] - M0;
    if constexpr (CLAMP) { a0 = mn(a0, lim); b0 = mn(b0, lim); a1 = mn(a1, lim); b1 = mn(b1, lim); }
    R[24] = mn(a0, b0); R[25] = mn(a1, b1);
    if constexpr (TIE == 1) fold<4>(acc1, sg(a0 - b0, a1 - b1)); else fold<4>(acc1, sg(b0 - a0, b1 - a1)); }
  { s2 a0 = R[26] - M1, b0 = R[27] + M1, a1 = R[26] + M1, b1 = R[27] - M1;
    if constexpr (CLAMP) { a0 = mn(a0, lim); b0 = mn(b0, lim); a1 = mn(a1, lim); b1 = mn(b1, lim); }
    R[26] = mn(a0, b0); R[27] = mn(a1, b1);
    if constexpr (TIE == 1) fold<5>(acc1, sg(a0 - b0, a1 - b1)); else fold<5>(acc1, sg(b0 - a0, b1 - a1)); }
  { s2 a0 = R[28] + M2, b0 = R[29] - M2, a1 = R[28] - M2, b1 = R[29] + M2;
    if constexpr (CLAMP) { a0 = mn(a0, lim); b0 = mn(b0, lim); a1 = mn(a1, lim); b1 = mn(b1, lim); }
    R[28] = mn(a0, b0); R[29] = mn(a1, b1);
    if constexpr (TIE == 1) fold<6>(acc1, sg(a0 - b0, a1 - b1)); else fold<6>(acc1, sg(b0 - a0, b1 - a1)); }
  { s2 a0 = R[30] + M3, b0 = R[31] - M3, a1 = R[30] - M3, b1 = R[31] + M3;
    if constexpr (CLAMP) { a0 = mn(a0, lim); b0 = mn(b0, lim); a1 = mn(a1, lim); b1 = mn(b1, lim); }
    R[30] = mn(a0, b0); R[31] = mn(a1, b1);
    if constexpr (TIE == 1) fold<7>(acc1, sg(a0 - b0, a1 - b1)); else fold<7>(acc1, sg(b0 - a0, b1 - a1)); }
  if constexpr (TIE == 1) { acc0 = ~acc0; acc1 = ~acc1; }
}

}}
```

Before: 554,400.

## Fold recentring into first ACS step and streamline Viterbi decision packing and traceback

For the non-tie Viterbi path, the per-cycle subtraction of R[0] from all 32 packed metric registers is no longer a separate pass. It is folded into step0 by precomputing branch metrics offset by the reference. Decision-bit extraction replaces two perms plus an OR per pair with one ydiff-based perm and a bfi fold, and a constant XOR fixes the polarity. Traceback now shifts bits into a single accumulator via alignbit with a reordered lookup table and a byte swap, is unrolled by 18 with a three-deep prefetch, and cuts ALU work in the serial traceback.

```diff
diff --git a/dabstar_amd/csrc/vit_t.hip b/dabstar_amd/csrc/vit_t.hip
--- a/dabstar_amd/csrc/vit_t.hip
+++ b/dabstar_amd/csrc/vit_t.hip
@@ -225,8 +225,8 @@
 template <> struct VtTie<1> { static constexpr int LIMTOP = 2 * 65535, REN2 = 2 * 60000; };
 template <> struct VtTie<2> { static constexpr int LIMTOP = 2 * 32767, REN2 = 2 * 30000; };
 
-template <int C, int TIE = 0, bool CLAMP = false>
-__device__ __forceinline__ void vt_one(vt::s2 (&R)[32], const VtCycle &cy, int t, const VtDec &dec_lane, vt::s2 v2n, int &Coff)
+template <int C, int TIE = 0, bool CLAMP = false, bool RC = false>
+__device__ __forceinline__ void vt_one(vt::s2 (&R)[32], const VtCycle &cy, int t, const VtDec &dec_lane, vt::s2 v2n, int &Coff, vt::s2 ref)
 {
   unsigned w[4], b[4];
 #pragma unroll
@@ -246,7 +246,7 @@
       lim = vt::pk(l, l);
     }
   }
-  if constexpr (C == 0) { vt::bm0(w, b, v2n, M); vt::step0<TIE, CLAMP>(R, M, acc0, acc1, lim); }
+  if constexpr (C == 0) { vt::bm0(w, b, v2n, M); vt::step0<TIE, CLAMP, RC>(R, M, acc0, acc1, lim, ref); }
   else if constexpr (C == 1) { vt::bm1(w, b, v2n, M); vt::step1<TIE, CLAMP>(R, M, acc0, acc1, lim); }
   else if constexpr (C == 2) { vt::bm2(w, b, v2n, M); vt::step2<TIE, CLAMP>(R, M, acc0, acc1, lim); }
   else if constexpr (C == 3) { vt::bm3(w, b, v2n, M); vt::step3<TIE, CLAMP>(R, M, acc0, acc1, lim); }
@@ -261,20 +261,22 @@
   }
 }
 
-template <int TIE, bool CLAMP>
-__device__ __forceinline__ void vt_cycle6(vt::s2 (&R)[32], const VtCycle &cy, int t0, const VtDec &dec_lane, vt::s2 v2n, int &Coff)
-{
-  vt_one<0, TIE, CLAMP>(R, cy, t0 + 0, dec_lane, v2n, Coff);
-  vt_one<1, TIE, CLAMP>(R, cy, t0 + 1, dec_lane, v2n, Coff);
-  vt_one<2, TIE, CLAMP>(R, cy, t0 + 2, dec_lane, v2n, Coff);
-  vt_one<3, TIE, CLAMP>(R, cy, t0 + 3, dec_lane, v2n, Coff);
-  vt_one<4, TIE, CLAMP>(R, cy, t0 + 4, dec_lane, v2n, Coff);
-  vt_one<5, TIE, CLAMP>(R, cy, t0 + 5, dec_lane, v2n, Coff);
-}
-template <int TIE, bool ALWAYS_CLAMP>
-__device__ __forceinline__ void vt_cycle(vt::s2 (&R)[32], const VtCycle &cy, int t0, const VtDec &dec_lane, vt::s2 v2n, int &Coff)
-{
-  if constexpr (TIE == 0) vt_cycle6<0, false>(R, cy, t0, dec_lane, v2n, Coff);
+template <int TIE, bool CLAMP, bool RC = false>
+__device__ __forceinline__ void vt_cycle6(vt::s2 (&R)[32], const VtCycle &cy, int t0, const VtDec &dec_lane, vt::s2 v2n, int &Coff,
+                                          vt::s2 ref = vt::s2{0, 0})
+{
+  vt_one<0, TIE, CLAMP, RC>(R, cy, t0 + 0, dec_lane, v2n, Coff, ref);
+  vt_one<1, TIE, CLAMP>(R, cy, t0 + 1, dec_lane, v2n, Coff, ref);
+  vt_one<2, TIE, CLAMP>(R, cy, t0 + 2, dec_lane, v2n, Coff, ref);
+  vt_one<3, TIE, CLAMP>(R, cy, t0 + 3, dec_lane, v2n, Coff, ref);
+  vt_one<4, TIE, CLAMP>(R, cy, t0 + 4, dec_lane, v2n, Coff, ref);
+  vt_one<5, TIE, CLAMP>(R, cy, t0 + 5, dec_lane, v2n, Coff, ref);
+}
+template <int TIE, bool ALWAYS_CLAMP, bool RC = false>
+__device__ __forceinline__ void vt_cycle(vt::s2 (&R)[32], const VtCycle &cy, int t0, const VtDec &dec_lane, vt::s2 v2n, int &Coff,
+                                         vt::s2 ref = vt::s2{0, 0})
+{
+  if constexpr (TIE == 0) vt_cycle6<0, false, RC>(R, cy, t0, dec_lane, v2n, Coff, ref);
   else {
     bool clamp = ALWAYS_CLAMP;
     if constexpr (!ALWAYS_CLAMP) {
@@ -299,21 +301,27 @@
   return d;
 }
 template <int C>
-__device__ __forceinline__ void vt_back_one(const uint2 w, int t, unsigned &L, unsigned &outw, uint32_t *out, const uint32_t *prbs,
-                                            const unsigned char *pos_c)
-{
-  constexpr unsigned p = 5 - C;
-  const unsigned pos = pos_c[L];
+__device__ __forceinline__ void vt_back_one(const uint2 w, int t, unsigned &acc, uint32_t *out, const uint32_t *prbs,
+                                            const unsigned char *bk_c)
+{
+  const unsigned pos = bk_c[acc >> 26];
   const unsigned long long ww = ((unsigned long long)w.y << 32) | w.x;
-  const unsigned bit = (unsigned)(ww >> pos) & 1u;
+  acc = __builtin_amdgcn_alignbit((unsigned)(ww >> pos), acc, 1u);
   const int qb = t - 6;
-  outw |= bit << (((qb >> 3) & 3) * 8 + 7 - (qb & 7));
-  L = (L & ~(1u << p)) | (bit << p);
   if ((qb & 31) == 0) {
     const unsigned pw = ((const __attribute__((address_space(4))) uint32_t *)(const void *)prbs)[qb >> 5];
-    if (out) out[qb >> 5] = outw ^ pw;
-    outw = 0;
-  }
+    if (out) out[qb >> 5] = __builtin_bswap32(acc) ^ pw;
+  }
+}
+__device__ __forceinline__ void vt_back6(const VtDec6 &d, int tc, unsigned &acc, uint32_t *out, const uint32_t *prbs,
+                                         const unsigned char (*bk)[64])
+{
+  vt_back_one<5>(d.w5, tc + 5, acc, out, prbs, bk[5]);
+  vt_back_one<4>(d.w4, tc + 4, acc, out, prbs, bk[4]);
+  vt_back_one<3>(d.w3, tc + 3, acc, out, prbs, bk[3]);
+  vt_back_one<2>(d.w2, tc + 2, acc, out, prbs, bk[2]);
+  vt_back_one<1>(d.w1, tc + 1, acc, out, prbs, bk[1]);
+  vt_back_one<0>(d.w0, tc + 0, acc, out, prbs, bk[0]);
 }
 
 __device__ unsigned long long *g_vt_timeline = nullptr;
@@ -322,7 +330,7 @@
 
 template <int TIE, bool ALWAYS_CLAMP>
 __device__ __forceinline__ void vt_decode(vt_rsrc in_grp, vt_cmap cmap, int nsteps, const VtDec &dec_lane, uint32_t *out, const uint32_t *prbs,
-                                          const unsigned char (*pos_tab)[64], int lane, unsigned long long &t_forward_end, bool want_time)
+                                          const unsigned char (*bk_tab)[64], int lane, unsigned long long &t_forward_end, bool want_time)
 {
   vt::s2 R[32];
 #pragma unroll
@@ -335,54 +343,57 @@
   vt_fetch(cb, in_grp, lane, cmap, 6);
   auto recentre = [&]() {
     const vt::s2 ref = vt::pk(R[0].x, R[0].x);
-    if constexpr (TIE != 0) Coff += (int)R[0].x;
-#pragma unroll
-    for (int r = 0; r < 32; r++) R[r] = R[r] - ref;
+    if constexpr (TIE != 0) {
+      Coff += (int)R[0].x;
+#pragma unroll
+      for (int r = 0; r < 32; r++) R[r] = R[r] - ref;
+    }
+    return ref;
   };
   vt::s2 v2n;
   asm volatile("v_mov_b32 %0, %1" : "=v"(v2n) : "s"(0xFFFE0002u));
   int t = 0;
   for (; t + 12 <= nsteps; t += 12) {
-    recentre();
-    vt_cycle<TIE, ALWAYS_CLAMP>(R, ca, t, dec_lane, v2n, Coff);
+    const vt::s2 ref = recentre();
+    vt_cycle<TIE, ALWAYS_CLAMP, TIE == 0>(R, ca, t, dec_lane, v2n, Coff, ref);
     vt_fetch(ca, in_grp, lane, cmap, t + 12 < last ? t + 12 : last);
     vt_cycle<TIE, ALWAYS_CLAMP>(R, cb, t + 6, dec_lane, v2n, Coff);
     vt_fetch(cb, in_grp, lane, cmap, t + 18 < last ? t + 18 : last);
   }
   if (t < nsteps) {
-    recentre();
-    vt_cycle<TIE, ALWAYS_CLAMP>(R, ca, t, dec_lane, v2n, Coff);
+    const vt::s2 ref = recentre();
+    vt_cycle<TIE, ALWAYS_CLAMP, TIE == 0>(R, ca, t, dec_lane, v2n, Coff, ref);
   }
   __builtin_amdgcn_fence(__ATOMIC_RELEASE, "workgroup");
   __builtin_amdgcn_s_waitcnt(0);
   __syncthreads();
   if (want_time) t_forward_end = __builtin_amdgcn_s_memrealtime();
 
-  unsigned L = 0, outw = 0;
-  VtDec6 cur = vt_load_dec(dec_lane, nsteps - 6);
-  VtDec6 nx1 = vt_load_dec(dec_lane, nsteps - 12);
-  for (int tc = nsteps - 6; tc >= 6; tc -= 6) {
-    const int tf = tc - 12 > 6 ? tc - 12 : 6;
-    const VtDec6 nx2 = vt_load_dec(dec_lane, tf);
-    vt_back_one<5>(cur.w5, tc + 5, L, outw, out, prbs, pos_tab[5]);
-    vt_back_one<4>(cur.w4, tc + 4, L, outw, out, prbs, pos_tab[4]);
-    vt_back_one<3>(cur.w3, tc + 3, L, outw, out, prbs, pos_tab[3]);
-    vt_back_one<2>(cur.w2, tc + 2, L, outw, out, prbs, pos_tab[2]);
-    vt_back_one<1>(cur.w1, tc + 1, L, outw, out, prbs, pos_tab[1]);
-    vt_back_one<0>(cur.w0, tc + 0, L, outw, out, prbs, pos_tab[0]);
-    cur = nx1; nx1 = nx2;
-  }
+  unsigned acc = 0;
+  VtDec6 da = vt_load_dec(dec_lane, nsteps - 6), db = vt_load_dec(dec_lane, nsteps - 12), dc;
+  auto ahead = [&](int tf) { return vt_load_dec(dec_lane, tf > 6 ? tf : 6); };
+  int tc = nsteps - 6;
+  for (; tc >= 18; tc -= 18) {
+    dc = ahead(tc - 12);
+    vt_back6(da, tc, acc, out, prbs, bk_tab);
+    da = ahead(tc - 18);
+    vt_back6(db, tc - 6, acc, out, prbs, bk_tab);
+    db = ahead(tc - 24);
+    vt_back6(dc, tc - 12, acc, out, prbs, bk_tab);
+  }
+  if (tc >= 6) vt_back6(da, tc, acc, out, prbs, bk_tab);
+  if (tc >= 12) vt_back6(db, tc - 6, acc, out, prbs, bk_tab);
 }
 
 template <int TIE>
 __device__ __forceinline__ void msc_vitT_body(const EngineDev &e, int cifs, const MscLaunch &ML, const uint32_t *prbs)
 {
-  __shared__ unsigned char pos_tab[6][64];
+  __shared__ unsigned char bk_tab[6][64];
   const int lane = threadIdx.x;
   unsigned long long *const tl = g_vt_timeline;
   unsigned long long tl0 = 0, tl1 = 0;
   if (tl) tl0 = __builtin_amdgcn_s_memrealtime();
-  for (int i = lane; i < 6 * 64; i += 64) pos_tab[i / 64][i % 64] = vt::VT_POS[i / 64][i % 64];
+  for (int i = lane; i < 6 * 64; i += 64) bk_tab[i / 64][i % 64] = vt::VT_BK[i / 64][i % 64];
   int gg = blockIdx.x;
   {
     constexpr int ROUND = 1024;
@@ -400,7 +411,7 @@
   uint32_t *out = nullptr;
   if (q.valid)
     out = reinterpret_cast<uint32_t *>(e.msc_out + (((size_t)q.s * e.max_subch + q.j) * MSC_SLOTS + (size_t)(q.out_idx % MSC_SLOTS)) * e.msc_stride);
-  vt_decode<TIE, false>(in_grp, cmap, nsteps, dec_lane, out, prbs, pos_tab, lane, tl1, tl != nullptr);
+  vt_decode<TIE, false>(in_grp, cmap, nsteps, dec_lane, out, prbs, bk_tab, lane, tl1, tl != nullptr);
   if (tl && lane == 0) {
     const unsigned slot = atomicAdd(&g_vt_timeline_n, 1u);
     if (slot < g_vt_timeline_cap) {
@@ -424,14 +435,14 @@
 template <int TIE, bool ALWAYS_CLAMP>
 __global__ __launch_bounds__(64) void k_vitT_stage(const uint32_t *symT, const uint16_t *map, int nbits, uint2 *decT, uint32_t *outw, const uint32_t *zeros)
 {
-  __shared__ unsigned char pos_tab[6][64];
+  __shared__ unsigned char bk_tab[6][64];
   const int lane = threadIdx.x, g = blockIdx.x;
-  for (int i = lane; i < 6 * 64; i += 64) pos_tab[i / 64][i % 64] = vt::VT_POS[i / 64][i % 64];
+  for (int i = lane; i < 6 * 64; i += 64) bk_tab[i / 64][i % 64] = vt::VT_BK[i / 64][i % 64];
   const int nsteps = nbits + 6, rows = nsteps + 1;
   const vt_rsrc in_grp = vt_make_rsrc(symT + (size_t)g * rows * 64, (unsigned)rows * 256u);
   unsigned long long unused = 0;
   vt_decode<TIE, ALWAYS_CLAMP>(in_grp, (vt_cmap)(const void *)map, nsteps, vt_make_dec(decT + (size_t)g * nsteps * 64, nsteps, lane),
-                               outw + ((size_t)g * 64 + lane) * (nbits / 32), zeros, pos_tab, lane, unused, false);
+                               outw + ((size_t)g * 64 + lane) * (nbits / 32), zeros, bk_tab, lane, unused, false);
 }
 
 extern "C" int dabx_internal_vitT(const int16_t *soft, int nbits, int batch, int tie_mode, int always_clamp, uint8_t *bits)
diff --git a/dabstar_amd/csrc/vit_t_gen.h b/dabstar_amd/csrc/vit_t_gen.h
--- a/dabstar_amd/csrc/vit_t_gen.h
+++ b/dabstar_amd/csrc/vit_t_gen.h
@@ -24,12 +24,13 @@
 __device__ __forceinline__ s2 sub_lh(s2 a, s2 b)
 { s2 r; asm("v_pk_sub_i16 %0, %1, %2 op_sel:[0,1] op_sel_hi:[1,0]" : "=v"(r) : "v"(a), "v"(b)); return r; }
 __device__ __forceinline__ unsigned sg(s2 s0, s2 s1) { return __builtin_amdgcn_perm(u(s0), u(s1), 0x0B0A0908u); }
-__device__ __forceinline__ unsigned sg_even(s2 dd, s2 ee) { return __builtin_amdgcn_perm(u(dd), u(ee), 0x0C0C090Au); }
-__device__ __forceinline__ unsigned sg_odd(s2 dd, s2 ee) { return __builtin_amdgcn_perm(u(dd), u(ee), 0x090A0C0Cu); }
 template <int K> __device__ __forceinline__ void fold(unsigned &acc, unsigned p)
 { constexpr unsigned M = 0x01010101u << K;
-  if (K == 0) acc = p & M;
-  else asm("v_and_or_b32 %0, %1, %2, %0" : "+v"(acc) : "v"(p), "s"(M)); }
+  if (K == 0) acc = p;
+  else asm("v_bfi_b32 %0, %1, %2, %0" : "+v"(acc) : "s"(M), "v"(p)); }
+__device__ __forceinline__ s2 ydiff(s2 t2, s2 t1) { return sub_hl(t2, t1) - s(0x00010000u); }
+__device__ __forceinline__ s2 ydiff_t1(s2 t1, s2 t2) { return sub_lh(t1, t2) - s(0x00010000u); }
+constexpr unsigned C0_INV = 0xFF00FF00u;
 __device__ __forceinline__ s2 swap_add(s2 a)
 { s2 r; asm("v_pk_add_u16 %0, %1, %1 op_sel:[0,1] op_sel_hi:[1,0]" : "=v"(r) : "v"(a)); return r; }
 __device__ __forceinline__ s2 swap_sub(s2 a) { return sub_lh(a, a); }
@@ -45,13 +46,12 @@
 { return s(__builtin_amdgcn_perm(w_hi, w_lo, 0x0C000C00u | b_lo | ((4u + b_hi) << 16))); }
 constexpr unsigned K_M255 = 0xFF01FF01u, K_M255_P255 = 0x00FFFF01u, K_M510 = 0xFE02FE02u, K_M510_P510 = 0x01FEFE02u;
 
-__device__ constexpr unsigned char VT_P[6] = {5, 4, 3, 2, 1, 0};
-__device__ constexpr unsigned char VT_POS[6][64] = {
-  {0, 16, 1, 17, 2, 18, 3, 19, 4, 20, 5, 21, 6, 22, 7, 23, 32, 48, 33, 49, 34, 50, 35, 51, 36, 52, 37, 53, 38, 54, 39, 55, 8, 24, 9, 25, 10, 26, 11, 27, 12, 28, 13, 29, 14, 30, 15, 31, 40, 56, 41, 57, 42, 58, 43, 59, 44, 60, 45, 61, 46, 62, 47, 63},
-  {16, 17, 18, 19, 20, 21, 22, 23, 48, 49, 50, 51, 52, 53, 54, 55, 0, 1, 2, 3, 4, 5, 6, 7, 32, 33, 34, 35, 36, 37, 38, 39, 24, 25, 26, 27, 28, 29, 30, 31, 56, 57, 58, 59, 60, 61, 62, 63, 8, 9, 10, 11, 12, 13, 14, 15, 40, 41, 42, 43, 44, 45, 46, 47},
-  {16, 17, 18, 19, 20, 21, 22, 23, 0, 1, 2, 3, 4, 5, 6, 7, 48, 49, 50, 51, 52, 53, 54, 55, 32, 33, 34, 35, 36, 37, 38, 39, 24, 25, 26, 27, 28, 29, 30, 31, 8, 9, 10, 11, 12, 13, 14, 15, 56, 57, 58, 59, 60, 61, 62, 63, 40, 41, 42, 43, 44, 45, 46, 47},
-  {16, 17, 18, 19, 0, 1, 2, 3, 20, 21, 22, 23, 4, 5, 6, 7, 48, 49, 50, 51, 32, 33, 34, 35, 52, 53, 54, 55, 36, 37, 38, 39, 24, 25, 26, 27, 8, 9, 10, 11, 28, 29, 30, 31, 12, 13, 14, 15, 56, 57, 58, 59, 40, 41, 42, 43, 60, 61, 62, 63, 44, 45, 46, 47},
-  {16, 17, 0, 1, 18, 19, 2, 3, 20, 21, 4, 5, 22, 23, 6, 7, 48, 49, 32, 33, 50, 51, 34, 35, 52, 53, 36, 37, 54, 55, 38, 39, 24, 25, 8, 9, 26, 27, 10, 11, 28, 29, 12, 13, 30, 31, 14, 15, 56, 57, 40, 41, 58, 59, 42, 43, 60, 61, 44, 45, 62, 63, 46, 47},
+__device__ constexpr unsigned char VT_BK[6][64] = {
+  {0, 8, 16, 24, 1, 9, 17, 25, 2, 10, 18, 26, 3, 11, 19, 27, 4, 12, 20, 28, 5, 13, 21, 29, 6, 14, 22, 30, 7, 15, 23, 31, 32, 40, 48, 56, 33, 41, 49, 57, 34, 42, 50, 58, 35, 43, 51, 59, 36, 44, 52, 60, 37, 45, 53, 61, 38, 46, 54, 62, 39, 47, 55, 63},
+  {16, 0, 24, 8, 17, 1, 25, 9, 18, 2, 26, 10, 19, 3, 27, 11, 20, 4, 28, 12, 21, 5, 29, 13, 22, 6, 30, 14, 23, 7, 31, 15, 48, 32, 56, 40, 49, 33, 57, 41, 50, 34, 58, 42, 51, 35, 59, 43, 52, 36, 60, 44, 53, 37, 61, 45, 54, 38, 62, 46, 55, 39, 63, 47},
+  {16, 0, 48, 32, 24, 8, 56, 40, 17, 1, 49, 33, 25, 9, 57, 41, 18, 2, 50, 34, 26, 10, 58, 42, 19, 3, 51, 35, 27, 11, 59, 43, 20, 4, 52, 36, 28, 12, 60, 44, 21, 5, 53, 37, 29, 13, 61, 45, 22, 6, 54, 38, 30, 14, 62, 46, 23, 7, 55, 39, 31, 15, 63, 47},
+  {16, 0, 20, 4, 48, 32, 52, 36, 24, 8, 28, 12, 56, 40, 60, 44, 17, 1, 21, 5, 49, 33, 53, 37, 25, 9, 29, 13, 57, 41, 61, 45, 18, 2, 22, 6, 50, 34, 54, 38, 26, 10, 30, 14, 58, 42, 62, 46, 19, 3, 23, 7, 51, 35, 55, 39, 27, 11, 31, 15, 59, 43, 63, 47},
+  {16, 0, 18, 2, 20, 4, 22, 6, 48, 32, 50, 34, 52, 36, 54, 38, 24, 8, 26, 10, 28, 12, 30, 14, 56, 40, 58, 42, 60, 44, 62, 46, 17, 1, 19, 3, 21, 5, 23, 7, 49, 33, 51, 35, 53, 37, 55, 39, 25, 9, 27, 11, 29, 13, 31, 15, 57, 41, 59, 43, 61, 45, 63, 47},
   {16, 0, 17, 1, 18, 2, 19, 3, 20, 4, 21, 5, 22, 6, 23, 7, 48, 32, 49, 33, 50, 34, 51, 35, 52, 36, 53, 37, 54, 38, 55, 39, 24, 8, 25, 9, 26, 10, 27, 11, 28, 12, 29, 13, 30, 14, 31, 15, 56, 40, 57, 41, 58, 42, 59, 43, 60, 44, 61, 45, 62, 46, 63, 47},
 };
 
@@ -69,142 +69,205 @@
   M[2] = add_hihi(Y2, D);
   M[3] = Y2 - S;
 }
-template <int TIE = 0, bool CLAMP = false>
-__device__ __forceinline__ void step0(s2 (&R)[32], const s2 (&M)[4], unsigned &acc0, unsigned &acc1, s2 lim = s2{0, 0})
-{
-  const s2 M0 = M[0];
-  const s2 M1 = M[1];
-  const s2 M2 = M[2];
-  const s2 M3 = M[3];
-  s2 t1_0 = R[0] + M0, t2_0 = R[0] - M0;
+template <int TIE = 0, bool CLAMP = false, bool RC = false>
+__device__ __forceinline__ void step0(s2 (&R)[32], const s2 (&M)[4], unsigned &acc0, unsigned &acc1, s2 lim = s2{0, 0}, s2 ref = s2{0, 0})
+{
+  s2 P[4], N[4];
+  if constexpr (RC) { const s2 nref = s2{0, 0} - ref; for (int i = 0; i < 4; i++) { P[i] = M[i] - ref; N[i] = nref - M[i]; } }
+  s2 t1_0, t2_0;
+  if constexpr (RC) { t1_0 = R[0] + P[0]; t2_0 = R[0] + N[0]; }
+  else { t1_0 = R[0] + M[0]; t2_0 = R[0] - M[0]; }
   if constexpr (CLAMP) { t1_0 = mn(t1_0, lim); t2_0 = mn(t2_0, lim); }
   R[0] = mn_x(t1_0, t2_0);
-  s2 t1_1 = R[1] + M3, t2_1 = R[1] - M3;
+  s2 t1_1, t2_1;
+  if constexpr (RC) { t1_1 = R[1] + P[3]; t2_1 = R[1] + N[3]; }
+  else { t1_1 = R[1] + M[3]; t2_1 = R[1] - M[3]; }
   if constexpr (CLAMP) { t1_1 = mn(t1_1, lim); t2_1 = mn(t2_1, lim); }
   R[1] = mn_x(t1_1, t2_1);
-  if constexpr (TIE == 1) fold<0>(acc0, sg_even(sub_lh(t1_0, t2_0), sub_hl(t2_0, t1_0)) | sg_odd(sub_lh(t1_1, t2_1), sub_hl(t2_1, t1_1)));
-  else fold<0>(acc0, sg_even(sub_hl(t2_0, t1_0), sub_lh(t1_0, t2_0)) | sg_odd(sub_hl(t2_1, t1_1), sub_lh(t1_1, t2_1)));
-  s2 t1_2 = R[2] - M1, t2_2 = R[2] + M1;
+  if constexpr (TIE == 1) fold<0>(acc0, sg(ydiff_t1(t1_1, t2_1), ydiff_t1(t1_0, t2_0)));
+  else fold<0>(acc0, sg(ydiff(t2_1, t1_1), ydiff(t2_0, t1_0)));
+  s2 t1_2, t2_2;
+  if constexpr (RC) { t1_2 = R[2] + N[1]; t2_2 = R[2] + P[1]; }
+  else { t1_2 = R[2] - M[1]; t2_2 = R[2] + M[1]; }
   if constexpr (CLAMP) { t1_2 = mn(t1_2, lim); t2_2 = mn(t2_2, lim); }
   R[2] = mn_x(t1_2, t2_2);
-  s2 t1_3 = R[3] - M2, t2_3 = R[3] + M2;
+  s2 t1_3, t2_3;
+  if constexpr (RC) { t1_3 = R[3] + N[2]; t2_3 = R[3] + P[2]; }
+  else { t1_3 = R[3] - M[2]; t2_3 = R[3] + M[2]; }
   if constexpr (CLAMP) { t1_3 = mn(t1_3, lim); t2_3 = mn(t2_3, lim); }
   R[3] = mn_x(t1_3, t2_3);
-  if constexpr (TIE == 1) fold<1>(acc0, sg_even(sub_lh(t1_2, t2_2), sub_hl(t2_2, t1_2)) | sg_odd(sub_lh(t1_3, t2_3), sub_hl(t2_3, t1_3)));
-  else fold<1>(acc0, sg_even(sub_hl(t2_2, t1_2), sub_lh(t1_2, t2_2)) | sg_odd(sub_hl(t2_3, t1_3), sub_lh(t1_3, t2_3)));
-  s2 t1_4 = R[4] - M1, t2_4 = R[4] + M1;
+  if constexpr (TIE == 1) fold<1>(acc0, sg(ydiff_t1(t1_3, t2_3), ydiff_t1(t1_2, t2_2)));
+  else fold<1>(acc0, sg(ydiff(t2_3, t1_3), ydiff(t2_2, t1_2)));
+  s2 t1_4, t2_4;
+  if constexpr (RC) { t1_4 = R[4] + N[1]; t2_4 = R[4] + P[1]; }
+  else { t1_4 = R[4] - M[1]; t2_4 = R[4] + M[1]; }
   if constexpr (CLAMP) { t1_4 = mn(t1_4, lim); t2_4 = mn(t2_4, lim); }
   R[4] = mn_x(t1_4, t2_4);
-  s2 t1_5 = R[5] - M2, t2_5 = R[5] + M2;
+  s2 t1_5, t2_5;
+  if constexpr (RC) { t1_5 = R[5] + N[2]; t2_5 = R[5] + P[2]; }
+  else { t1_5 = R[5] - M[2]; t2_5 = R[5] + M[2]; }
   if constexpr (CLAMP) { t1_5 = mn(t1_5, lim); t2_5 = mn(t2_5, lim); }
   R[5] = mn_x(t1_5, t2_5);
-  if constexpr (TIE == 1) fold<2>(acc0, sg_even(sub_lh(t1_4, t2_4), sub_hl(t2_4, t1_4)) | sg_odd(sub_lh(t1_5, t2_5), sub_hl(t2_5, t1_5)));
-  else fold<2>(acc0, sg_even(sub_hl(t2_4, t1_4), sub_lh(t1_4, t2_4)) | sg_odd(sub_hl(t2_5, t1_5), sub_lh(t1_5, t2_5)));
-  s2 t1_6 = R[6] + M0, t2_6 = R[6] - M0;
+  if constexpr (TIE == 1) fold<2>(acc0, sg(ydiff_t1(t1_5, t2_5), ydiff_t1(t1_4, t2_4)));
+  else fold<2>(acc0, sg(ydiff(t2_5, t1_5), ydiff(t2_4, t1_4)));
+  s2 t1_6, t2_6;
+  if constexpr (RC) { t1_6 = R[6] + P[0]; t2_6 = R[6] + N[0]; }
+  else { t1_6 = R[6] + M[0]; t2_6 = R[6] - M[0]; }
   if constexpr (CLAMP) { t1_6 = mn(t1_6, lim); t2_6 = mn(t2_6, lim); }
   R[6] = mn_x(t1_6, t2_6);
-  s2 t1_7 = R[7] + M3, t2_7 = R[7] - M3;
+  s2 t1_7, t2_7;
+  if constexpr (RC) { t1_7 = R[7] + P[3]; t2_7 = R[7] + N[3]; }
+  else { t1_7 = R[7] + M[3]; t2_7 = R[7] - M[3]; }
   if constexpr (CLAMP) { t1_7 = mn(t1_7, lim); t2_7 = mn(t2_7, lim); }
   R[7] = mn_x(t1_7, t2_7);
-  if constexpr (TIE == 1) fold<3>(acc0, sg_even(sub_lh(t1_6, t2_6), sub_hl(t2_6, t1_6)) | sg_odd(sub_lh(t1_7, t2_7), sub_hl(t2_7, t1_7)));
-  else fold<3>(acc0, sg_even(sub_hl(t2_6, t1_6), sub_lh(t1_6, t2_6)) | sg_odd(sub_hl(t2_7, t1_7), sub_lh(t1_7, t2_7)));
-  s2 t1_8 = R[8] + M1, t2_8 = R[8] - M1;
+  if constexpr (TIE == 1) fold<3>(acc0, sg(ydiff_t1(t1_7, t2_7), ydiff_t1(t1_6, t2_6)));
+  else fold<3>(acc0, sg(ydiff(t2_7, t1_7), ydiff(t2_6, t1_6)));
+  s2 t1_8, t2_8;
+  if constexpr (RC) { t1_8 = R[8] + P[1]; t2_8 = R[8] + N[1]; }
+  else { t1_8 = R[8] + M[1]; t2_8 = R[8] - M[1]; }
   if constexpr (CLAMP) { t1_8 = mn(t1_8, lim); t2_8 = mn(t2_8, lim); }
   R[8] = mn_x(t1_8, t2_8);
-  s2 t1_9 = R[9] + M2, t2_9 = R[9] - M2;
+  s2 t1_9, t2_9;
+  if constexpr (RC) { t1_9 = R[9] + P[2]; t2_9 = R[9] + N[2]; }
+  else { t1_9 = R[9] + M[2]; t2_9 = R[9] - M[2]; }
   if constexpr (CLAMP) { t1_9 = mn(t1_9, lim); t2_9 = mn(t2_9, lim); }
   R[9] = mn_x(t1_9, t2_9);
-  if constexpr (TIE == 1) fold<4>(acc0, sg_even(sub_lh(t1_8, t2_8), sub_hl(t2_8, t1_8)) | sg_odd(sub_lh(t1_9, t2_9), sub_hl(t2_9, t1_9)));
-  else fold<4>(acc0, sg_even(sub_hl(t2_8, t1_8), sub_lh(t1_8, t2_8)) | sg_odd(sub_hl(t2_9, t1_9), sub_lh(t1_9, t2_9)));
-  s2 t1_10 = R[10] - M0, t2_10 = R[10] + M0;
+  if constexpr (TIE == 1) fold<4>(acc0, sg(ydiff_t1(t1_9, t2_9), ydiff_t1(t1_8, t2_8)));
+  else fold<4>(acc0, sg(ydiff(t2_9, t1_9), ydiff(t2_8, t1_8)));
+  s2 t1_10, t2_10;
+  if constexpr (RC) { t1_10 = R[10] + N[0]; t2_10 = R[10] + P[0]; }
+  else { t1_10 = R[10] - M[0]; t2_10 = R[10] + M[0]; }
   if constexpr (CLAMP) { t1_10 = mn(t1_10, lim); t2_10 = mn(t2_10, lim); }
   R[10] = mn_x(t1_10, t2_10);
-  s2 t1_11 = R[11] - M3, t2_11 = R[11] + M3;
+  s2 t1_11, t2_11;
+  if constexpr (RC) { t1_11 = R[11] + N[3]; t2_11 = R[11] + P[3]; }
+  else { t1_11 = R[11] - M[3]; t2_11 = R[11] + M[3]; }
   if constexpr (CLAMP) { t1_11 = mn(t1_11, lim); t2_11 = mn(t2_11, lim); }
   R[11] = mn_x(t1_11, t2_11);
-  if constexpr (TIE == 1) fold<5>(acc0, sg_even(sub_lh(t1_10, t2_10), sub_hl(t2_10, t1_10)) | sg_odd(sub_lh(t1_11, t2_11), sub_hl(t2_11, t1_11)));
-  else fold<5>(acc0, sg_even(sub_hl(t2_10, t1_10), sub_lh(t1_10, t2_10)) | sg_odd(sub_hl(t2_11, t1_11), sub_lh(t1_11, t2_11)));
-  s2 t1_12 = R[12] - M0, t2_12 = R[12] + M0;
+  if constexpr (TIE == 1) fold<5>(acc0, sg(ydiff_t1(t1_11, t2_11), ydiff_t1(t1_10, t2_10)));
+  else fold<5>(acc0, sg(ydiff(t2_11, t1_11), ydiff(t2_10, t1_10)));
+  s2 t1_12, t2_12;
+  if constexpr (RC) { t1_12 = R[12] + N[0]; t2_12 = R[12] + P[0]; }
+  else { t1_12 = R[12] - M[0]; t2_12 = R[12] + M[0]; }
   if constexpr (CLAMP) { t1_12 = mn(t1_12, lim); t2_12 = mn(t2_12, lim); }
   R[12] = mn_x(t1_12, t2_12);
-  s2 t1_13 = R[13] - M3, t2_13 = R[13] + M3;
+  s2 t1_13, t2_13;
+  if constexpr (RC) { t1_13 = R[13] + N[3]; t2_13 = R[13] + P[3]; }
+  else { t1_13 = R[13] - M[3]; t2_13 = R[13] + M[3]; }
   if constexpr (CLAMP) { t1_13 = mn(t1_13, lim); t2_13 = mn(t2_13, lim); }
   R[13] = mn_x(t1_13, t2_13);
-  if constexpr (TIE == 1) fold<6>(acc0, sg_even(sub_lh(t1_12, t2_12), sub_hl(t2_12, t1_12)) | sg_odd(sub_lh(t1_13, t2_13), sub_hl(t2_13, t1_13)));
-  else fold<6>(acc0, sg_even(sub_hl(t2_12, t1_12), sub_lh(t1_12, t2_12)) | sg_odd(sub_hl(t2_13, t1_13), sub_lh(t1_13, t2_13)));
-  s2 t1_14 = R[14] + M1, t2_14 = R[14] - M1;
+  if constexpr (TIE == 1) fold<6>(acc0, sg(ydiff_t1(t1_13, t2_13), ydiff_t1(t1_12, t2_12)));
+  else fold<6>(acc0, sg(ydiff(t2_13, t1_13), ydiff(t2_12, t1_12)));
+  s2 t1_14, t2_14;
+  if constexpr (RC) { t1_14 = R[14] + P[1]; t2_14 = R[14] + N[1]; }
+  else { t1_14 = R[14] + M[1]; t2_14 = R[14] - M[1]; }
   if constexpr (CLAMP) { t1_14 = mn(t1_14, lim); t2_14 = mn(t2_14, lim); }
   R[14] = mn_x(t1_14, t2_14);
-  s2 t1_15 = R[15] + M2, t2_15 = R[15] - M2;
+  s2 t1_15, t2_15;
+  if constexpr (RC) { t1_15 = R[15] + P[2]; t2_15 = R[15] + N[2]; }
+  else { t1_15 = R[15] + M[2]; t2_15 = R[15] - M[2]; }
   if constexpr (CLAMP) { t1_15 = mn(t1_15, lim); t2_15 = mn(t2_15, lim); }
   R[15] = mn_x(t1_15, t2_15);
-  if constexpr (TIE == 1) fold<7>(acc0, sg_even(sub_lh(t1_14, t2_14), sub_hl(t2_14, t1_14)) | sg_odd(sub_lh(t1_15, t2_15), sub_hl(t2_15, t1_15)));
-  else fold<7>(acc0, sg_even(sub_hl(t2_14, t1_14), sub_lh(t1_14, t2_14)) | sg_odd(sub_hl(t2_15, t1_15), sub_lh(t1_15, t2_15)));
-  s2 t1_16 = R[16] - M3, t2_16 = R[16] + M3;
+  if constexpr (TIE == 1) fold<7>(acc0, sg(ydiff_t1(t1_15, t2_15), ydiff_t1(t1_14, t2_14)));
+  else fold<7>(acc0, sg(ydiff(t2_15, t1_15), ydiff(t2_14, t1_14)));
+  s2 t1_16, t2_16;
+  if constexpr (RC) { t1_16 = R[16] + N[3]; t2_16 = R[16] + P[3]; }
+  else { t1_16 = R[16] - M[3]; t2_16 = R[16] + M[3]; }
   if constexpr (CLAMP) { t1_16 = mn(t1_16, lim); t2_16 = mn(t2_16, lim); }
   R[16] = mn_x(t1_16, t2_16);
-  s2 t1_17 = R[17] - M0, t2_17 = R[17] + M0;
+  s2 t1_17, t2_17;
+  if constexpr (RC) { t1_17 = R[17] + N[0]; t2_17 = R[17] + P[0]; }
+  else { t1_17 = R[17] - M[0]; t2_17 = R[17] + M[0]; }
   if constexpr (CLAMP) { t1_17 = mn(t1_17, lim); t2_17 = mn(t2_17, lim); }
   R[17] = mn_x(t1_17, t2_17);
-  if constexpr (TIE == 1) fold<0>(acc1, sg_even(sub_lh(t1_16, t2_16), sub_hl(t2_16, t1_16)) | sg_odd(sub_lh(t1_17, t2_17), sub_hl(t2_17, t1_17)));
-  else fold<0>(acc1, sg_even(sub_hl(t2_16, t1_16), sub_lh(t1_16, t2_16)) | sg_odd(sub_hl(t2_17, t1_17), sub_lh(t1_17, t2_17)));
-  s2 t1_18 = R[18] + M2, t2_18 = R[18] - M2;
+  if constexpr (TIE == 1) fold<0>(acc1, sg(ydiff_t1(t1_17, t2_17), ydiff_t1(t1_16, t2_16)));
+  else fold<0>(acc1, sg(ydiff(t2_17, t1_17), ydiff(t2_16, t1_16)));
+  s2 t1_18, t2_18;
+  if constexpr (RC) { t1_18 = R[18] + P[2]; t2_18 = R[18] + N[2]; }
+  else { t1_18 = R[18] + M[2]; t2_18 = R[18] - M[2]; }
   if constexpr (CLAMP) { t1_18 = mn(t1_18, lim); t2_18 = mn(t2_18, lim); }
   R[18] = mn_x(t1_18, t2_18);
-  s2 t1_19 = R[19] + M1, t2_19 = R[19] - M1;
+  s2 t1_19, t2_19;
+  if constexpr (RC) { t1_19 = R[19] + P[1]; t2_19 = R[19] + N[1]; }
+  else { t1_19 = R[19] + M[1]; t2_19 = R[19] - M[1]; }
   if constexpr (CLAMP) { t1_19 = mn(t1_19, lim); t2_19 = mn(t2_19, lim); }
   R[19] = mn_x(t1_19, t2_19);
-  if constexpr (TIE == 1) fold<1>(acc1, sg_even(sub_lh(t1_18, t2_18), sub_hl(t2_18, t1_18)) | sg_odd(sub_lh(t1_19, t2_19), sub_hl(t2_19, t1_19)));
-  else fold<1>(acc1, sg_even(sub_hl(t2_18, t1_18), sub_lh(t1_18, t2_18)) | sg_odd(sub_hl(t2_19, t1_19), sub_lh(t1_19, t2_19)));
-  s2 t1_20 = R[20] + M2, t2_20 = R[20] - M2;
+  if constexpr (TIE == 1) fold<1>(acc1, sg(ydiff_t1(t1_19, t2_19), ydiff_t1(t1_18, t2_18)));
+  else fold<1>(acc1, sg(ydiff(t2_19, t1_19), ydiff(t2_18, t1_18)));
+  s2 t1_20, t2_20;
+  if constexpr (RC) { t1_20 = R[20] + P[2]; t2_20 = R[20] + N[2]; }
+  else { t1_20 = R[20] + M[2]; t2_20 = R[20] - M[2]; }
   if constexpr (CLAMP) { t1_20 = mn(t1_20, lim); t2_20 = mn(t2_20, lim); }
   R[20] = mn_x(t1_20, t2_20);
-  s2 t1_21 = R[21] + M1, t2_21 = R[21] - M1;
+  s2 t1_21, t2_21;
+  if constexpr (RC) { t1_21 = R[21] + P[1]; t2_21 = R[21] + N[1]; }
+  else { t1_21 = R[21] + M[1]; t2_21 = R[21] - M[1]; }
   if constexpr (CLAMP) { t1_21 = mn(t1_21, lim); t2_21 = mn(t2_21, lim); }
   R[21] = mn_x(t1_21, t2_21);
-  if constexpr (TIE == 1) fold<2>(acc1, sg_even(sub_lh(t1_20, t2_20), sub_hl(t2_20, t1_20)) | sg_odd(sub_lh(t1_21, t2_21), sub_hl(t2_21, t1_21)));
-  else fold<2>(acc1, sg_even(sub_hl(t2_20, t1_20), sub_lh(t1_20, t2_20)) | sg_odd(sub_hl(t2_21, t1_21), sub_lh(t1_21, t2_21)));
-  s2 t1_22 = R[22] - M3, t2_22 = R[22] + M3;
+  if constexpr (TIE == 1) fold<2>(acc1, sg(ydiff_t1(t1_21, t2_21), ydiff_t1(t1_20, t2_20)));
+  else fold<2>(acc1, sg(ydiff(t2_21, t1_21), ydiff(t2_20, t1_20)));
+  s2 t1_22, t2_22;
+  if constexpr (RC) { t1_22 = R[22] + N[3]; t2_22 = R[22] + P[3]; }
+  else { t1_22 = R[22] - M[3]; t2_22 = R[22] + M[3]; }
   if constexpr (CLAMP) { t1_22 = mn(t1_22, lim); t2_22 = mn(t2_22, lim); }
   R[22] = mn_x(t1_22, t2_22);
-  s2 t1_23 = R[23] - M0, t2_23 = R[23] + M0;
+  s2 t1_23, t2_23;
+  if constexpr (RC) { t1_23 = R[23] + N[0]; t2_23 = R[23] + P[0]; }
+  else { t1_23 = R[23] - M[0]; t2_23 = R[23] + M[0]; }
   if constexpr (CLAMP) { t1_23 = mn(t1_23, lim); t2_23 = mn(t2_23, lim); }
   R[23] = mn_x(t1_23, t2_23);
-  if constexpr (TIE == 1) fold<3>(acc1, sg_even(sub_lh(t1_22, t2_22), sub_hl(t2_22, t1_22)) | sg_odd(sub_lh(t1_23, t2_23), sub_hl(t2_23, t1_23)));
-  else fold<3>(acc1, sg_even(sub_hl(t2_22, t1_22), sub_lh(t1_22, t2_22)) | sg_odd(sub_hl(t2_23, t1_23), sub_lh(t1_23, t2_23)));
-  s2 t1_24 = R[24] - M2, t2_24 = R[24] + M2;
+  if constexpr (TIE == 1) fold<3>(acc1, sg(ydiff_t1(t1_23, t2_23), ydiff_t1(t1_22, t2_22)));
+  else fold<3>(acc1, sg(ydiff(t2_23, t1_23), ydiff(t2_22, t1_22)));
+  s2 t1_24, t2_24;
+  if constexpr (RC) { t1_24 = R[24] + N[2]; t2_24 = R[24] + P[2]; }
+  else { t1_24 = R[24] - M[2]; t2_24 = R[24] + M[2]; }
   if constexpr (CLAMP) { t1_24 = mn(t1_24, lim); t2_24 = mn(t2_24, lim); }
   R[24] = mn_x(t1_24, t2_24);
-  s2 t1_25 = R[25] - M1, t2_25 = R[25] + M1;
+  s2 t1_25, t2_25;
+  if constexpr (RC) { t1_25 = R[25] + N[1]; t2_25 = R[25] + P[1]; }
+  else { t1_25 = R[25] - M[1]; t2_25 = R[25] + M[1]; }
   if constexpr (CLAMP) { t1_25 = mn(t1_25, lim); t2_25 = mn(t2_25, lim); }
   R[25] = mn_x(t1_25, t2_25);
-  if constexpr (TIE == 1) fold<4>(acc1, sg_even(sub_lh(t1_24, t2_24), sub_hl(t2_24, t1_24)) | sg_odd(sub_lh(t1_25, t2_25), sub_hl(t2_25, t1_25)));
-  else fold<4>(acc1, sg_even(sub_hl(t2_24, t1_24), sub_lh(t1_24, t2_24)) | sg_odd(sub_hl(t2_25, t1_25), sub_lh(t1_25, t2_25)));
-  s2 t1_26 = R[26] + M3, t2_26 = R[26] - M3;
+  if constexpr (TIE == 1) fold<4>(acc1, sg(ydiff_t1(t1_25, t2_25), ydiff_t1(t1_24, t2_24)));
+  else fold<4>(acc1, sg(ydiff(t2_25, t1_25), ydiff(t2_24, t1_24)));
+  s2 t1_26, t2_26;
+  if constexpr (RC) { t1_26 = R[26] + P[3]; t2_26 = R[26] + N[3]; }
+  else { t1_26 = R[26] + M[3]; t2_26 = R[26] - M[3]; }
   if constexpr (CLAMP) { t1_26 = mn(t1_26, lim); t2_26 = mn(t2_26, lim); }
   R[26] = mn_x(t1_26, t2_26);
-  s2 t1_27 = R[27] + M0, t2_27 = R[27] - M0;
+  s2 t1_27, t2_27;
+  if constexpr (RC) { t1_27 = R[27] + P[0]; t2_27 = R[27] + N[0]; }
+  else { t1_27 = R[27] + M[0]; t2_27 = R[27] - M[0]; }
   if constexpr (CLAMP) { t1_27 = mn(t1_27, lim); t2_27 = mn(t2_27, lim); }
   R[27] = mn_x(t1_27, t2_27);
-  if constexpr (TIE == 1) fold<5>(acc1, sg_even(sub_lh(t1_26, t2_26), sub_hl(t2_26, t1_26)) | sg_odd(sub_lh(t1_27, t2_27), sub_hl(t2_27, t1_27)));
-  else fold<5>(acc1, sg_even(sub_hl(t2_26, t1_26), sub_lh(t1_26, t2_26)) | sg_odd(sub_hl(t2_27, t1_27), sub_lh(t1_27, t2_27)));
-  s2 t1_28 = R[28] + M3, t2_28 = R[28] - M3;
+  if constexpr (TIE == 1) fold<5>(acc1, sg(ydiff_t1(t1_27, t2_27), ydiff_t1(t1_26, t2_26)));
+  else fold<5>(acc1, sg(ydiff(t2_27, t1_27), ydiff(t2_26, t1_26)));
+  s2 t1_28, t2_28;
+  if constexpr (RC) { t1_28 = R[28] + P[3]; t2_28 = R[28] + N[3]; }
+  else { t1_28 = R[28] + M[3]; t2_28 = R[28] - M[3]; }
   if constexpr (CLAMP) { t1_28 = mn(t1_28, lim); t2_28 = mn(t2_28, lim); }
   R[28] = mn_x(t1_28, t2_28);
-  s2 t1_29 = R[29] + M0, t2_29 = R[29] - M0;
+  s2 t1_29, t2_29;
+  if constexpr (RC) { t1_29 = R[29] + P[0]; t2_29 = R[29] + N[0]; }
+  else { t1_29 = R[29] + M[0]; t2_29 = R[29] - M[0]; }
   if constexpr (CLAMP) { t1_29 = mn(t1_29, lim); t2_29 = mn(t2_29, lim); }
   R[29] = mn_x(t1_29, t2_29);
-  if constexpr (TIE == 1) fold<6>(acc1, sg_even(sub_lh(t1_28, t2_28), sub_hl(t2_28, t1_28)) | sg_odd(sub_lh(t1_29, t2_29), sub_hl(t2_29, t1_29)));
-  else fold<6>(acc1, sg_even(sub_hl(t2_28, t1_28), sub_lh(t1_28, t2_28)) | sg_odd(sub_hl(t2_29, t1_29), sub_lh(t1_29, t2_29)));
-  s2 t1_30 = R[30] - M2, t2_30 = R[30] + M2;
+  if constexpr (TIE == 1) fold<6>(acc1, sg(ydiff_t1(t1_29, t2_29), ydiff_t1(t1_28, t2_28)));
+  else fold<6>(acc1, sg(ydiff(t2_29, t1_29), ydiff(t2_28, t1_28)));
+  s2 t1_30, t2_30;
+  if constexpr (RC) { t1_30 = R[30] + N[2]; t2_30 = R[30] + P[2]; }
+  else { t1_30 = R[30] - M[2]; t2_30 = R[30] + M[2]; }
   if constexpr (CLAMP) { t1_30 = mn(t1_30, lim); t2_30 = mn(t2_30, lim); }
   R[30] = mn_x(t1_30, t2_30);
-  s2 t1_31 = R[31] - M1, t2_31 = R[31] + M1;
+  s2 t1_31, t2_31;
+  if constexpr (RC) { t1_31 = R[31] + N[1]; t2_31 = R[31] + P[1]; }
+  else { t1_31 = R[31] - M[1]; t2_31 = R[31] + M[1]; }
   if constexpr (CLAMP) { t1_31 = mn(t1_31, lim); t2_31 = mn(t2_31, lim); }
   R[31] = mn_x(t1_31, t2_31);
-  if constexpr (TIE == 1) fold<7>(acc1, sg_even(sub_lh(t1_30, t2_30), sub_hl(t2_30, t1_30)) | sg_odd(sub_lh(t1_31, t2_31), sub_hl(t2_31, t1_31)));
-  else fold<7>(acc1, sg_even(sub_hl(t2_30, t1_30), sub_lh(t1_30, t2_30)) | sg_odd(sub_hl(t2_31, t1_31), sub_lh(t1_31, t2_31)));
-  if constexpr (TIE == 1) { acc0 = ~acc0; acc1 = ~acc1; }
+  if constexpr (TIE == 1) fold<7>(acc1, sg(ydiff_t1(t1_31, t2_31), ydiff_t1(t1_30, t2_30)));
+  else fold<7>(acc1, sg(ydiff(t2_31, t1_31), ydiff(t2_30, t1_30)));
+  if constexpr (TIE == 1) { acc0 ^= ~C0_INV; acc1 ^= ~C0_INV; }
+  else { acc0 ^= C0_INV; acc1 ^= C0_INV; }
 }
 
 __device__ __forceinline__ void bm1(const unsigned (&w)[4], const unsigned (&b)[4], s2 v2n, s2 (&M)[4])
```

Result: faster. 562,800, median of 6 (+1.5%).
